# DeltaPavonis/cpp_raytracer

Hardware: AMD Instinct MI355X
Metric: Msamples/sec + achieved HBM GB/s, RTOW final scene at 1/2/4/8 MI355X (higher is better)
Workload: dtype f64; 1 GPU; rtow_final seed 42, 1200x800, 500 spp, max_depth 50 (BASELINE config 2); primitives=485, bvh_nodes=115, partition=whole frame on one GPU

## Files before the change

### cpp_raytracer_amd/__init__.py

```python
from __future__ import annotations

import ctypes as C
import struct
from dataclasses import dataclass
from pathlib import Path
from typing import Optional

import numpy as np

from . import _capi
from ._capi import (CRT_BOX, CRT_DIELECTRIC, CRT_DIFFUSE_LIGHT, CRT_LAMBERTIAN, CRT_METAL,
                    CRT_PARALLELOGRAM, CRT_SPHERE, HIT_DTYPE, MATERIAL_DTYPE, NODE_DTYPE,
                    OBJECT_DTYPE, CRT_BLOCK_STOPPED, FEATURE_DTYPE, BVHParams, Camera, CameraSettings, CrtError,
                    DenoiseParams, RenderStats, SceneInfo, Tiling, TraceParams, CRT_TRACE_ANY, CRT_TRACE_PLAIN,
                    RadianceParams, CRT_RADIANCE_PLAIN, ProbeParams, CRT_PROBE_SPHERE, CRT_PROBE_HEMISPHERE,
                    CRT_SH_RADIANCE, CRT_SH_IRRADIANCE, Lens, CRT_LENS_PINHOLE, CRT_LENS_ORTHOGRAPHIC,
                    CRT_LENS_EQUIRECT, CRT_LENS_FISHEYE, CRT_LENS_CUBE, check, lib)

__all__ = [
    "SceneData", "GpuScene", "CameraSettings", "Camera", "Tiling", "RenderStats", "CrtError",
    "resolve_camera", "sample_seed", "rand_double", "device_count", "lib", "ppm_values", "write_ppm",
    "sample_chunk_len", "noise_estimate", "block_count", "adaptive_update", "CRT_BLOCK_STOPPED",
    "DenoiseParams", "FEATURE_DTYPE", "denoise_params", "pixel_variance", "denoise",
    "TraceParams", "CRT_TRACE_ANY", "CRT_TRACE_PLAIN", "HIT_DTYPE",
# ... 174 lines not shown
    def save(self, path) -> None:
        Path(path).write_bytes(self.to_bytes())

    @classmethod
    def from_bytes(cls, b: bytes) -> "SceneData":
        if b[:4] != SCENE_MAGIC:
            raise CrtError("not a CRTS scene file")
        ver, nm, no = struct.unpack_from("<IQQ", b, 4)
        if ver != SCENE_VERSION:
            raise CrtError(f"CRTS version {ver} unsupported")
        off = 4 + struct.calcsize("<IQQ")
        cs = CameraSettings.from_buffer_copy(b[off:off + C.sizeof(CameraSettings)])
        off += C.sizeof(CameraSettings)
        mats = np.frombuffer(b, MATERIAL_DTYPE, nm, off).copy()
        off += nm * MATERIAL_DTYPE.itemsize
        objs = np.frombuffer(b, OBJECT_DTYPE, no, off).copy()
        return cls(mats, objs, cs)

    @classmethod
    def load(cls, path) -> "SceneData":
        return cls.from_bytes(Path(path).read_bytes())


def resolve_camera(settings: CameraSettings, base_seed: int = 0) -> Camera:
    cam = Camera()
    check(lib().crt_camera_resolve(C.byref(settings), C.byref(cam)), "crt_camera_resolve")
    cam.base_seed = base_seed & 0xFFFFFFFF
    return cam


def camera_with(settings: CameraSettings, **kw) -> CameraSettings:
    cs = CameraSettings.from_buffer_copy(_settings_bytes(settings))
    for k, v in kw.items():
        setattr(cs, k, v)
    return cs


class GpuScene:

    def __init__(self, data: SceneData, num_buckets: int = 32, max_prims_in_node: int = 12,
                 linear: bool = False, build_device: Optional[int] = None):
        self.data = data
        self._h = C.c_void_p()
        mats = np.ascontiguousarray(data.materials, dtype=MATERIAL_DTYPE)
        objs = np.ascontiguousarray(data.objects, dtype=OBJECT_DTYPE)
        prm = BVHParams(num_buckets, max_prims_in_node, int(linear),
                        0 if build_device is None else build_device + 1)
        check(lib().crt_scene_create(mats.ctypes.data, len(mats), objs.ctypes.data, len(objs),
                                     C.byref(prm), C.byref(self._h)), "crt_scene_create")

    def close(self) -> None:
        if self._h:
            lib().crt_scene_destroy(self._h)
            self._h = C.c_void_p()

    def __del__(self):
        try:
            self.close()
        except Exception:
            pass

    @property
    def handle(self) -> C.c_void_p:
        return self._h

    def info(self) -> SceneInfo:
        si = SceneInfo()
        check(lib().crt_scene_info_get(self._h, C.byref(si)), "crt_scene_info_get")
        return si

    def export_bvh(self) -> tuple[np.ndarray, np.ndarray]:
        si = self.info()
        nodes = np.zeros(si.num_nodes, NODE_DTYPE)
        order = np.zeros(si.num_primitives, np.uint32)
        check(lib().crt_scene_export_bvh(self._h, nodes.ctypes.data, order.ctypes.data),
              "crt_scene_export_bvh")
        return nodes, order

    def launch_plan(self, kernel="render") -> _capi.LaunchPlan:
        k = {"render": _capi.CRT_PLAN_RENDER, "trace": _capi.CRT_PLAN_TRACE, "radiance": _capi.CRT_PLAN_RADIANCE}.get(kernel, kernel)
        p = _capi.LaunchPlan()
        check(lib().crt_launch_plan(self._h, int(k), C.byref(p)), "crt_launch_plan")
        return p

    def upload(self, device: int = 0) -> None:
        check(lib().crt_scene_upload(self._h, device), f"crt_scene_upload(device={device})")

    def device_image(self, device: int = 0) -> np.ndarray:
        out = np.zeros(self.info().device_bytes, np.uint8)
        check(lib().crt_scene_image(self._h, device, out.ctypes.data, out.nbytes),
              f"crt_scene_image(device={device})")
        return out

    def render_async(self, device: int, cam: Camera, out_ptr: int, stream: int = 0,
                     tiling: Optional[Tiling] = None) -> None:
        t = C.byref(tiling) if tiling is not None else None
        check(lib().crt_render_async(self._h, device, C.byref(cam), t, C.c_void_p(out_ptr),
                                     C.c_void_p(stream)), "crt_render_async")

    def render_pass(self, device: int, cam: Camera, first: int, count: int, sum_ptr: int,
                    noise_ptr: int = 0, out_ptr: int = 0, stream: int = 0,
                    tiling: Optional[Tiling] = None) -> None:
        t = C.byref(tiling) if tiling is not None else None
        check(lib().crt_render_pass_async(self._h, device, C.byref(cam), t, first, count,
                                          C.c_void_p(sum_ptr), C.c_void_p(noise_ptr or None),
                                          C.c_void_p(out_ptr or None), C.c_void_p(stream)),
              "crt_render_pass_async")

    def render_pass_masked(self, device: int, cam: Camera, first: int, count: int, sum_ptr: int,
                           noise_ptr: int, out_ptr: int, blocks_ptr: int, active_hint: int = 0,
                           stream: int = 0, tiling: Optional[Tiling] = None) -> None:
        t = C.byref(tiling) if tiling is not None else None
        check(lib().crt_render_pass_masked_async(self._h, device, C.byref(cam), t, first, count,
                                                 C.c_void_p(sum_ptr), C.c_void_p(noise_ptr or None),
                                                 C.c_void_p(out_ptr or None), C.c_void_p(blocks_ptr or None),
                                                 min(active_hint, 0xFFFFFFFF), C.c_void_p(stream)),
              "crt_render_pass_masked_async")

    def render_adaptive(self, cam: Camera, threshold: float, min_samples: int = 0, samples_per_pass: int = 0,
                        callback=None, num_devices: int = 1,
                        preview: bool = False) -> tuple[np.ndarray, np.ndarray, int]:
        out = np.empty((cam.image_h, cam.image_w, 3), np.float64)
        counts = np.zeros(((cam.image_h + 3) // 4, (cam.image_w + 15) // 16), np.uint32)
        raised = []

        def trampoline(_user, done, total, active, blocks, h_rgb):
            try:
                return 1 if callback(done, total, active, blocks, out if h_rgb else None) else 0
            except BaseException as e:
                raised.append(e)
                return 1

        fn = _capi.ADAPTIVE_FN(trampoline) if callback is not None else _capi.ADAPTIVE_FN()
        prm = _capi.AdaptiveParams(threshold, min_samples, samples_per_pass,
                                   _capi.CRT_PROGRESS_PREVIEW if preview else 0, 0)
        rendered = C.c_uint64(0)
        rc = lib().crt_render_adaptive(self._h, C.byref(cam), num_devices, C.byref(prm), fn, None,
                                       out.ctypes.data, counts.ctypes.data, C.byref(rendered))
        if raised:
            raise raised[0]
        check(rc, "crt_render_adaptive")
        return out, counts, int(rendered.value)

    adaptive_update = staticmethod(adaptive_update)
    block_count = staticmethod(block_count)
    pixel_variance = staticmethod(pixel_variance)
    denoise = staticmethod(denoise)

    def render_features(self, device: int, cam: Camera, feat_ptr: int, stream: int = 0,
                        tiling: Optional[Tiling] = None) -> None:
        t = C.byref(tiling) if tiling is not None else None
        check(lib().crt_render_features_async(self._h, device, C.byref(cam), t, C.c_void_p(feat_ptr or None),
                                              C.c_void_p(stream)), "crt_render_features_async")

    def render_denoised(self, cam: Camera, params: Optional[DenoiseParams] = None, threshold: Optional[float] = None,
                        min_samples: int = 0, samples_per_pass: int = 0, device: int = 0,
                        noisy: bool = False, *, num_devices: int = 1, callback=None, preview: bool = False,
                        counts: bool = False):
        out = np.empty((cam.image_h, cam.image_w, 3), np.float64)
        raw = np.empty_like(out) if noisy else None
        prm = params if params is not None else denoise_params()
        rendered = C.c_uint64(0)
        if num_devices == 1 and callback is None and not preview and not counts:
            ad = _capi.AdaptiveParams(threshold, min_samples, samples_per_pass, 0, 0) if threshold is not None else None
            check(lib().crt_render_denoised(self._h, device, C.byref(cam), C.byref(ad) if ad is not None else None,
                                            C.byref(prm), raw.ctypes.data if noisy else None, out.ctypes.data,
# ... 357 lines not shown
```

### cpp_raytracer_amd/_capi.py

```python
from __future__ import annotations

import ctypes as C
import os
from pathlib import Path

import numpy as np

PKG_DIR = Path(__file__).resolve().parent
LIB_PATH = Path(os.environ.get("CRT_LIB", PKG_DIR / "lib" / "libcrt_hip.so"))

CRT_LAMBERTIAN, CRT_METAL, CRT_DIELECTRIC, CRT_DIFFUSE_LIGHT = 1, 2, 3, 4
CRT_SPHERE, CRT_PARALLELOGRAM, CRT_BOX = 1, 2, 3

D3 = C.c_double * 3


class Material(C.Structure):
    _fields_ = [("kind", C.c_uint32), ("reserved", C.c_uint32), ("color", D3), ("param", C.c_double)]


class Object(C.Structure):
    _fields_ = [("kind", C.c_uint32), ("material", C.c_uint32), ("v", C.c_double * 9)]


# ... 142 lines not shown
ADAPTIVE_FN = C.CFUNCTYPE(C.c_int, C.c_void_p, C.c_uint32, C.c_uint32, C.c_uint32, C.c_uint32, C.c_void_p)
DENOISED_FN = C.CFUNCTYPE(C.c_int, C.c_void_p, C.c_uint32, C.c_uint32, C.c_uint32, C.c_uint32, C.c_void_p, C.c_void_p)
CRT_BLOCK_W, CRT_BLOCK_H, CRT_BLOCK_STOPPED = 16, 4, 0x80000000
EXPORTS = {
    "crt_abi_version": (C.c_int, []),
    "crt_last_error": (C.c_char_p, []),
    "crt_build_info": (C.c_char_p, []),
    "crt_device_count": (C.c_int, [P(C.c_int)]),
    "crt_free": (None, [C.c_void_p]),
    "crt_sample_seed": (C.c_uint32, [C.c_uint32, C.c_uint32, C.c_uint32]),
    "crt_rand_double": (C.c_double, [P(C.c_uint32), C.c_double, C.c_double]),
    "crt_scene_build_named": (C.c_int, [C.c_char_p, C.c_uint32, C.c_int, P(P(Material)), P(C.c_size_t),
                                        P(P(Object)), P(C.c_size_t), P(CameraSettings)]),
    "crt_scene_create": (C.c_int, [C.c_void_p, C.c_size_t, C.c_void_p, C.c_size_t, P(BVHParams),
                                   P(C.c_void_p)]),
    "crt_scene_info_get": (C.c_int, [C.c_void_p, P(SceneInfo)]),
    "crt_scene_export_bvh": (C.c_int, [C.c_void_p, C.c_void_p, C.c_void_p]),
    "crt_scene_upload": (C.c_int, [C.c_void_p, C.c_int]),
    "crt_scene_image": (C.c_int, [C.c_void_p, C.c_int, C.c_void_p, C.c_size_t]),
    "crt_scene_destroy": (None, [C.c_void_p]),
    "crt_camera_resolve": (C.c_int, [P(CameraSettings), P(Camera)]),
    "crt_render_async": (C.c_int, [C.c_void_p, C.c_int, P(Camera), P(Tiling), C.c_void_p, C.c_void_p]),
    "crt_sample_chunk_len": (C.c_uint32, [C.c_uint32]),
    "crt_render_pass_async": (C.c_int, [C.c_void_p, C.c_int, P(Camera), P(Tiling), C.c_uint32, C.c_uint32,
                                        C.c_void_p, C.c_void_p, C.c_void_p, C.c_void_p]),
    "crt_noise_estimate": (C.c_int, [C.c_int, C.c_void_p, C.c_size_t, C.c_uint32, C.c_uint32,
                                     P(C.c_double), P(C.c_double), C.c_void_p]),
    "crt_render_progressive": (C.c_int, [C.c_void_p, P(Camera), C.c_int, C.c_uint32, C.c_uint32, PROGRESS_FN,
                                         C.c_void_p, C.c_void_p, P(C.c_uint32)]),
    "crt_block_count": (C.c_size_t, [C.c_uint32, C.c_uint32]),
    "crt_render_pass_masked_async": (C.c_int, [C.c_void_p, C.c_int, P(Camera), P(Tiling), C.c_uint32, C.c_uint32,
                                               C.c_void_p, C.c_void_p, C.c_void_p, C.c_void_p, C.c_uint32,
                                               C.c_void_p]),
    "crt_adaptive_update": (C.c_int, [C.c_int, P(Camera), P(Tiling), C.c_void_p, C.c_void_p, C.c_uint32,
                                      C.c_double, C.c_uint32, P(C.c_uint32), C.c_void_p]),
    "crt_render_adaptive": (C.c_int, [C.c_void_p, P(Camera), C.c_int, P(AdaptiveParams), ADAPTIVE_FN, C.c_void_p,
                                      C.c_void_p, C.c_void_p, P(C.c_uint64)]),
    "crt_render_features_async": (C.c_int, [C.c_void_p, C.c_int, P(Camera), P(Tiling), C.c_void_p, C.c_void_p]),
    "crt_pixel_variance_async": (C.c_int, [C.c_int, P(Camera), P(Tiling), C.c_void_p, C.c_void_p, C.c_uint32,
                                           C.c_void_p, C.c_void_p]),
    "crt_denoise_async": (C.c_int, [C.c_int, C.c_uint32, C.c_uint32, C.c_void_p, C.c_void_p, C.c_void_p,
                                    P(DenoiseParams), C.c_void_p, C.c_void_p, C.c_void_p]),
    "crt_render_denoised": (C.c_int, [C.c_void_p, C.c_int, P(Camera), P(AdaptiveParams), P(DenoiseParams),
                                      C.c_void_p, C.c_void_p, P(C.c_uint64)]),
    "crt_render_denoised_devices": (C.c_int, [C.c_void_p, P(Camera), C.c_int, P(AdaptiveParams), P(DenoiseParams),
                                              DENOISED_FN, C.c_void_p, C.c_void_p, C.c_void_p, C.c_void_p,
                                              P(C.c_uint64)]),
    "crt_render_count": (C.c_int, [C.c_void_p, C.c_int, P(Camera), P(Tiling), P(RenderStats)]),
    "crt_render": (C.c_int, [C.c_void_p, P(Camera), C.c_int, C.c_void_p, P(RenderStats)]),
    "crt_render_ppm": (C.c_int, [C.c_void_p, P(Camera), C.c_int, C.c_void_p, P(RenderStats)]),
    "crt_closest_hits": (C.c_int, [C.c_void_p, C.c_int, C.c_void_p, C.c_size_t, C.c_double, C.c_double,
                                   C.c_void_p]),
    "crt_trace_async": (C.c_int, [C.c_void_p, C.c_int, C.c_void_p, C.c_size_t, C.c_void_p, P(TraceParams),
                                  C.c_void_p, C.c_void_p, C.c_void_p]),
    "crt_trace": (C.c_int, [C.c_void_p, C.c_int, C.c_void_p, C.c_size_t, C.c_void_p, P(TraceParams), C.c_void_p,
                            C.c_void_p]),
    "crt_radiance_async": (C.c_int, [C.c_void_p, C.c_int, C.c_void_p, C.c_size_t, C.c_void_p, P(RadianceParams),
                                     C.c_void_p, C.c_void_p]),
    "crt_radiance": (C.c_int, [C.c_void_p, C.c_int, C.c_void_p, C.c_size_t, C.c_void_p, P(RadianceParams),
                               C.c_void_p]),
    "crt_camera_rays_async": (C.c_int, [C.c_int, P(Camera), P(Tiling), C.c_uint32, C.c_uint32, C.c_void_p,
                                        C.c_void_p, C.c_void_p]),
    "crt_probe_rays_async": (C.c_int, [C.c_int, C.c_void_p, C.c_void_p, C.c_size_t, P(ProbeParams), C.c_void_p,
                                       C.c_void_p, C.c_void_p]),
    "crt_probes_async": (C.c_int, [C.c_void_p, C.c_int, C.c_void_p, C.c_void_p, C.c_size_t, P(ProbeParams),
                                   C.c_void_p, C.c_void_p]),
    "crt_probes": (C.c_int, [C.c_void_p, C.c_int, C.c_void_p, C.c_void_p, C.c_size_t, P(ProbeParams), C.c_void_p]),
    "crt_sh_eval_async": (C.c_int, [C.c_int, C.c_void_p, C.c_size_t, C.c_void_p, C.c_void_p, C.c_size_t, C.c_uint32,
                                    C.c_void_p, C.c_void_p]),
    "crt_lens_rays_async": (C.c_int, [C.c_int, P(Camera), P(Lens), C.c_uint32, C.c_uint32, C.c_void_p, C.c_void_p,
                                      C.c_void_p]),
    "crt_render_lens_async": (C.c_int, [C.c_void_p, C.c_int, P(Camera), P(Lens), C.c_void_p, C.c_void_p]),
    "crt_render_lens": (C.c_int, [C.c_void_p, C.c_int, P(Camera), P(Lens), C.c_void_p]),
    "crt_render_lens_pass_async": (C.c_int, [C.c_void_p, C.c_int, P(Camera), P(Lens), C.c_uint32, C.c_uint32,
                                             C.c_void_p, C.c_void_p, C.c_void_p, C.c_void_p, C.c_uint32, C.c_void_p]),
    "crt_lens_centre_rays_async": (C.c_int, [C.c_int, P(Camera), P(Lens), C.c_void_p, C.c_void_p]),
    "crt_lens_features_async": (C.c_int, [C.c_void_p, C.c_int, P(Camera), P(Lens), C.c_void_p, C.c_void_p]),
    "crt_render_lens_passes": (C.c_int, [C.c_void_p, C.c_int, P(Camera), P(Lens), P(AdaptiveParams), P(DenoiseParams),
                                         DENOISED_FN, C.c_void_p, C.c_void_p, C.c_void_p, C.c_void_p, P(C.c_uint64)]),
    "crt_ppm_values": (C.c_int, [C.c_int, C.c_void_p, C.c_size_t, C.c_void_p, C.c_void_p]),
    "crt_ppm_write": (C.c_int, [C.c_char_p, C.c_uint32, C.c_uint32, C.c_void_p]),
    "crt_render_guard": (C.c_int, [C.c_void_p, C.c_int, P(C.c_uint64), C.c_int]),
    "crt_launch_plan": (C.c_int, [C.c_void_p, C.c_uint32, P(LaunchPlan)]),
}


class CrtError(RuntimeError):
    pass


_lib = None


def lib() -> C.CDLL:
    global _lib
    if _lib is None:
        if not LIB_PATH.exists():
            raise CrtError(f"{LIB_PATH} is missing: run __graft_entry__.build() "
                           "(make -C cpp_raytracer_amd); there is no fallback path")
        h = C.CDLL(str(LIB_PATH), mode=os.RTLD_NOW | C.RTLD_GLOBAL)
        for name, (res, args) in EXPORTS.items():
            f = getattr(h, name)
            f.restype = res
            f.argtypes = args
        _lib = h
    return _lib


def check(rc: int, what: str = "") -> None:
    if rc != 0:
        msg = lib().crt_last_error().decode(errors="replace")
        raise CrtError(f"{what or 'crt'} failed ({rc}): {msg}")
```

### cpp_raytracer_amd/csrc/crt_device.hip

```cpp
#include <hip/hip_runtime.h>

#define CRT_HD __host__ __device__ __forceinline__

#include <algorithm>
#include <atomic>
#include <cmath>
#include <cstdio>
#include <cstring>
#include <limits>
#include <string>
#include <mutex>
#include <thread>
#include <type_traits>
#include <vector>

#include "crt_internal.h"
#include "crt_hip_util.h"
#include "crt_rows.h"
#include "crt_ray_class.h"
#include "crt_schlick.h"

#pragma clang fp contract(off)

namespace crt {

namespace dev {

#ifndef CRT_BLOCK
#define CRT_BLOCK 256
#endif
constexpr int kBlock = CRT_BLOCK;
#ifndef CRT_TILE_W
#define CRT_TILE_W 16
#endif
constexpr uint32_t kTileW = CRT_TILE_W, kTileH = 64 / CRT_TILE_W;
constexpr int kManyWaves = 5;
#ifndef CRT_PAIR_WALK
#define CRT_PAIR_WALK 1
#endif
constexpr double kScale = 1 / static_cast<double>(4294967295u - 1);

typedef double Dvec2 __attribute__((ext_vector_type(2)));
typedef uint32_t Uvec4 __attribute__((ext_vector_type(4)));

struct SceneView {
    const DevNode* nodes;
    const DevNodeF* fnodes;
    uint32_t ntop;
    const uint32_t* refs;
    const DevSphere* spheres;
    const DevSpherePair* spair;
    uint32_t spair_lds;
    const uint32_t* sphere_mat;
    const DevQuad* quads;
    const uint32_t* quad_mat;
    const DevMaterial* mats;
    const DevQuadF* quadf;
    const DevMaterial* sphere_mrec;
    const DevMaterial* quad_mrec;
    uint32_t quadf_lds;
    const DevQuadBox* quadbox;
    uint32_t refs_lds, spheres_lds, quads_lds;
    uint32_t inv64_lds;
    unsigned long long* guard;
};

struct CamView {
    double o[3], p00[3], pdx[3], pdy[3], ddx[3], ddy[3];
    double defocus_angle;
    double bg[3];
    double t_min;
    double inv_spp;
    uint32_t w, h, spp, max_depth, base_seed;
};

struct Work {
    uint32_t owned_rows;
    uint32_t row_block, tile_count, tile_index;
    uint32_t col0, k0, bw, bh;
    uint32_t tiles_x, tiles_y, tiles;
    uint32_t chunks, chunk_len;
    uint32_t s0;
    uint32_t* queue;
    uint32_t segments;
    uint32_t n_items, bulk_items;
    uint32_t item_chunks, groups, bulk_chunks, tail_chunks;
    uint32_t rb_shift;
    uint32_t lds_nodes, lds_refs, lds_spheres, lds_quads, lds_quadf, lds_stack;
    uint32_t bytes_nodes, bytes_refs, bytes_spheres, bytes_quads, bytes_quadf;
    uint32_t lds_sph64, bytes_sph64;
    uint32_t sphere_only;
    uint32_t exact_slab;
    uint32_t ntop;
    uint32_t sentinel;
    uint32_t lds_cam;
    uint32_t lds_acc;
    uint32_t lds_inv64;
    uint32_t packed;
    uint32_t count_spec, round_counters;
    uint32_t f32_ok;
    uint32_t pair_walk;
    uint32_t spheres_f32;
    uint32_t quads_f32;
    uint32_t quads_flat;
    float tmin32;
};

struct Counters {
    unsigned long long rays, nodes, sphere_tests, quad_tests;
    unsigned long long cyc_walk, cyc_leaf, cyc_shade, cyc_total;
    unsigned long long cyc_tail;
    unsigned long long it_walk, it_leaf, it_shade;
    unsigned long long slow_nodes, it_slow;
    unsigned long long cand, it_cand;
    unsigned long long rounds, round_walkers, round_leaves, round_done, shade_rounds;
    unsigned long long cyc_draw, cyc_init;
};

struct LaneCounters {
    uint32_t rays, nodes, sphere_tests, quad_tests;
    uint32_t it_walk, it_leaf, it_shade;
    uint32_t slow_nodes, it_slow;
    uint32_t cand, it_cand;
};

__device__ __forceinline__ void flush_counts(LaneCounters& c, Counters* t) {
    using ull = unsigned long long;
    atomicAdd(&t->rays, static_cast<ull>(c.rays));
    atomicAdd(&t->nodes, static_cast<ull>(c.nodes));
    atomicAdd(&t->sphere_tests, static_cast<ull>(c.sphere_tests));
    atomicAdd(&t->quad_tests, static_cast<ull>(c.quad_tests));
    atomicAdd(&t->it_walk, static_cast<ull>(c.it_walk));
    atomicAdd(&t->it_leaf, static_cast<ull>(c.it_leaf));
    atomicAdd(&t->it_shade, static_cast<ull>(c.it_shade));
    atomicAdd(&t->slow_nodes, static_cast<ull>(c.slow_nodes));
    atomicAdd(&t->it_slow, static_cast<ull>(c.it_slow));
    atomicAdd(&t->cand, static_cast<ull>(c.cand));
    atomicAdd(&t->it_cand, static_cast<ull>(c.it_cand));
    c = LaneCounters{};
}

__device__ __forceinline__ bool wave_leader() {
    const uint64_t m = __ballot(1);
    return (threadIdx.x & 63) == static_cast<uint32_t>(__ffsll(static_cast<long long>(m)) - 1);
}

#ifndef CRT_WATCHDOG
#define CRT_WATCHDOG 0
#endif
#if CRT_WATCHDOG
__device__ unsigned long long crt_wd_deadline;
#define CRT_WD(id, a, b)                                                                                   \
    do {                                                                                                   \
        if (wall_clock64() > *(volatile unsigned long long*)&crt_wd_deadline) {                            \
            if (wave_leader())                                                                             \
                printf("crt watchdog: block %u wave %u loop %d a %u b %u\n", blockIdx.x, threadIdx.x >> 6,  \
                       (int)(id), (unsigned)(a), (unsigned)(b));                                            \
            __builtin_amdgcn_endpgm();                                                                     \
        }                                                                                                  \
    } while (0)
#else
#define CRT_WD(id, a, b) do {} while (0)
#endif

__device__ __forceinline__ double rnd(uint32_t& s, double lo, double hi) {
    s = 1664525u * s + 1013904223u;
    return lo + (hi - lo) * static_cast<double>(s) * kScale;
}
__device__ __forceinline__ double rnd_pm1(uint32_t& s) {
    s = 1664525u * s + 1013904223u;
    return static_cast<double>(s) * (2 * kScale) + -1.0;
}
__device__ __forceinline__ double rnd_01(uint32_t& s) {
    s = 1664525u * s + 1013904223u;
    return static_cast<double>(s) * kScale;
}

__device__ __forceinline__ uint32_t sample_seed(uint32_t base, uint32_t pixel, uint32_t sample) {
    uint64_t z = (static_cast<uint64_t>(pixel) << 32) | sample;
    z += static_cast<uint64_t>(base) * 0x9E3779B97F4A7C15ull;
// ... 538 lines not shown
__device__ __forceinline__ bool slab64_inv(GlobalNode* p, const double o[3], uint32_t inv_lds, double tmin,
                                           double tmax) {
    NodeLines nd;
    node_lines(p, nd);
    typedef __attribute__((address_space(3))) const double LdsDoubleC;
    uint32_t t = threadIdx.x;
    asm volatile("" : "+v"(t));
    LdsDoubleC* q = (LdsDoubleC*)static_cast<uintptr_t>(inv_lds + t * 8);
    const double inv[3] = {q[0], q[kBlock], q[2 * kBlock]};
    const Dvec2 bx = nd.b[0], by = nd.b[1], bz = nd.b[2];
    const double x0 = (bx.x - o[0]) * inv[0], x1 = (bx.y - o[0]) * inv[0];
    const double y0 = (by.x - o[1]) * inv[1], y1 = (by.y - o[1]) * inv[1];
    const double z0 = (bz.x - o[2]) * inv[2], z1 = (bz.y - o[2]) * inv[2];
    const double near = fmax(fmax(fmin(x0, x1), fmin(y0, y1)), fmin(z0, z1));
    const double far = fmin(fmin(fmax(x0, x1), fmax(y0, y1)), fmax(z0, z1));
    return (near <= far) & (near < tmax) & (far > tmin);
}

struct NodeF {
    Uvec4 q0;
    Uvec4 q1;
};
typedef __attribute__((address_space(3))) const NodeF LdsNodeF;
typedef __attribute__((address_space(1))) const NodeF GlobalNodeF;
template <bool TOP, bool LS>
__device__ __forceinline__ void fetch_nodef(const SceneView& S, uint32_t cur, Uvec4& q0, Uvec4& q1) {
    if (LS) {
        LdsNodeF* p = (LdsNodeF*)static_cast<uintptr_t>(cur);
        q0 = p->q0;
        q1 = p->q1;
    } else if (TOP) {
        const uint64_t hbm = __ballot(cur >= S.ntop);
        uint64_t save;
        asm volatile(
            "s_and_saveexec_b64 %[save], %[hbm]\n\t"
            "s_cbranch_execz 1f\n\t"
            "global_load_dwordx4 %[q0], %[cur], %[base]\n\t"
            "global_load_dwordx4 %[q1], %[cur], %[base] offset:16\n"
            "1:\n\t"
            "s_andn2_b64 exec, %[save], %[hbm]\n\t"
            "s_cbranch_execz 2f\n\t"
            "ds_read_b128 %[q0], %[cur]\n\t"
            "ds_read_b128 %[q1], %[cur] offset:16\n"
            "2:\n\t"
            "s_mov_b64 exec, %[save]\n\t"
            "s_waitcnt vmcnt(0) lgkmcnt(0)"
            : [q0] "=&v"(q0), [q1] "=&v"(q1), [save] "=&s"(save)
            : [cur] "v"(cur), [hbm] "s"(hbm), [base] "s"(S.fnodes)
            : "memory");
    } else {
        GlobalNodeF* p = (GlobalNodeF*)(reinterpret_cast<const char*>(S.fnodes) + cur);
        q0 = p->q0;
        q1 = p->q1;
    }
}

typedef uint32_t Uvec2 __attribute__((ext_vector_type(2)));
template <bool TOP, bool LS>
__device__ __forceinline__ Uvec2 fetch_nodef_words(const SceneView& S, uint32_t cur) {
    typedef __attribute__((address_space(3))) const Uvec2 LdsU2;
    typedef __attribute__((address_space(1))) const Uvec2 GlobalU2;
    if (LS) return *(LdsU2*)static_cast<uintptr_t>(cur + 24);
    if (!TOP) return *(GlobalU2*)(reinterpret_cast<const char*>(S.fnodes) + cur + 24);
    const uint64_t hbm = __ballot(cur >= S.ntop);
    uint64_t save;
    Uvec2 w;
    asm volatile(
        "s_and_saveexec_b64 %[save], %[hbm]\n\t"
        "s_cbranch_execz 1f\n\t"
        "global_load_dwordx2 %[w], %[cur], %[base] offset:24\n"
        "1:\n\t"
        "s_andn2_b64 exec, %[save], %[hbm]\n\t"
        "s_cbranch_execz 2f\n\t"
        "ds_read_b64 %[w], %[cur] offset:24\n"
        "2:\n\t"
        "s_mov_b64 exec, %[save]\n\t"
        "s_waitcnt vmcnt(0) lgkmcnt(0)"
        : [w] "=&v"(w), [save] "=&s"(save)
        : [cur] "v"(cur), [hbm] "s"(hbm), [base] "s"(S.fnodes)
        : "memory");
    return w;
}

template <typename SE, bool COUNT, bool EXACT, bool TOP, bool LS, bool GS, bool SPEC, bool INVL = false, bool G2 = true>
__device__ __forceinline__ void walk(const SceneView& S, Stack<SE>& st, const double o[3], const double d[3],
                                     double tmin, float tmin32, Trav& R, LaneCounters& ctr) {
    const ptrdiff_t stride = static_cast<ptrdiff_t>(st.stride);
    SE* const empty = st.base - stride;
    SE* tp = st.base + (static_cast<ptrdiff_t>(R.sp) - 1) * stride;
    uint32_t cur = R.cur;
    uint32_t w0, w1;
    bool stop;
    if (EXACT) {
        double dx = d[0], dy = d[1], dz = d[2];
        asm volatile("" : "+v"(dx), "+v"(dy), "+v"(dz));
        const double inv[3] = {1 / dx, 1 / dy, 1 / dz};
        do {
            NodeLines nd;
            node_lines(node64(S, cur), nd);
            const Uvec4 meta = nd.meta;
            const uint32_t top = *tp;
            if (COUNT) {
                if (meta.y != kSentinelCount) ctr.nodes++;
                if (wave_leader()) ctr.it_walk++;
            }
            const bool nx = R.neg & 1u, ny = (R.neg >> 1) & 1u, nz = (R.neg >> 2) & 1u;
            const double bx0 = nx ? nd.b[0].y : nd.b[0].x, bx1 = nx ? nd.b[0].x : nd.b[0].y;
            const double by0 = ny ? nd.b[1].y : nd.b[1].x, by1 = ny ? nd.b[1].x : nd.b[1].y;
            const double bz0 = nz ? nd.b[2].y : nd.b[2].x, bz1 = nz ? nd.b[2].x : nd.b[2].y;
            double xtmin = (bx0 - o[0]) * inv[0];
            double xtmax = (bx1 - o[0]) * inv[0];
            const double ytmin = (by0 - o[1]) * inv[1];
            const double ytmax = (by1 - o[1]) * inv[1];
            const double ztmin = (bz0 - o[2]) * inv[2];
            const double ztmax = (bz1 - o[2]) * inv[2];
            const bool c1 = !(xtmin > ytmax || ytmin > xtmax);
            if (ytmin > xtmin) xtmin = ytmin;
            if (ytmax < xtmax) xtmax = ytmax;
            const bool c2 = !(xtmin > ztmax || ztmin > xtmax);
            if (ztmin > xtmin) xtmin = ztmin;
            if (ztmax < xtmax) xtmax = ztmax;
            const bool enter = (c1 & c2 & (xtmin < R.tmax) & (xtmax > tmin)) |
                               (meta.y != 0 && (meta.w & kNodeAlways) != 0) | (meta.y == kSentinelCount);
            const bool inner = enter & (meta.y == 0);
            const bool far_first = (R.neg >> meta.z) & 1u;
            const uint32_t left = meta.w << kNodeFShift, right = meta.x << kNodeFShift;
            tp[stride] = static_cast<SE>(far_first ? left : right);
            stop = enter ^ inner;
            cur = inner ? (far_first ? right : left) : top;
            tp += inner ? stride : -stride;
            w0 = meta.x;
            w1 = meta.y == kSentinelCount ? kSentinelW1 : (kLeafFlagF | meta.y);
        } while (!stop);
    } else if (SPEC) {
        bool run = true, nopend = true;
        uint32_t pref = ~0u, pcur = 0;
        do {
            CRT_WD(4, cur, static_cast<uint32_t>(tp - empty));
            if (run) {
                Uvec4 q0, q1;
                fetch_nodef<TOP, LS>(S, cur, q0, q1);
                w0 = q1.z;
                w1 = q1.w;
                const uint32_t top = *tp;
                if (COUNT) {
                    if (w1 != kSentinelW1) ctr.nodes++;
                    if (wave_leader()) ctr.it_walk++;
                }
                const float x0 = __builtin_fmaf(__uint_as_float(q0.x), R.inv32[0], -R.oinv32[0]);
                const float x1 = __builtin_fmaf(__uint_as_float(q0.y), R.inv32[0], -R.oinv32[0]);
                const float y0 = __builtin_fmaf(__uint_as_float(q0.z), R.inv32[1], -R.oinv32[1]);
                const float y1 = __builtin_fmaf(__uint_as_float(q0.w), R.inv32[1], -R.oinv32[1]);
                const float z0 = __builtin_fmaf(__uint_as_float(q1.x), R.inv32[2], -R.oinv32[2]);
                const float z1 = __builtin_fmaf(__uint_as_float(q1.y), R.inv32[2], -R.oinv32[2]);
                const float lo = vmax3(vmin(x0, x1), vmin(y0, y1), vmax_s(vmin(z0, z1), tmin32));
                const float hi = vmin3(vmax(x0, x1), vmax(y0, y1), vmin(vmax(z0, z1), R.tmax32));
                const float gap = hi - lo;
                const float th = __builtin_fmaf(vmax_abs(lo, hi), 0x1p-19f, R.marg);
                bool enter = gap > 0.f;
                const bool unc = !(fabsf(gap) > th);
                if (__builtin_expect(__ballot(unc) != 0, 0)) {
                    if (COUNT && wave_leader()) ctr.it_slow++;
                    if (unc) {
                        if (COUNT) ctr.slow_nodes++;
                        enter = INVL ? slab64_inv(node64(S, cur), o, S.inv64_lds, tmin, R.tmax)
                                     : slab64(node64(S, cur), o, d, tmin, R.tmax);
                    }
                }
                const bool inner = enter & (w1 < kLeafFlagF);
                const uint32_t near = w1 | (__builtin_amdgcn_ubfe(R.neg, w0, 1) << kNodeFShift);
                tp[stride] = static_cast<SE>(near ^ (1u << kNodeFShift));
                const bool reached = enter & !inner;
                const bool park = reached & (!nopend | (!G2 && w1 == kSentinelW1));
                pref = (reached & nopend) ? cur : pref;
                pcur = park ? cur : pcur;
                run = !park;
                cur = inner ? near : top;
                tp += inner ? stride : -stride;
            }
            nopend = pref == ~0u;
        } while (__ballot(nopend) != 0);
        if (!run) {
            cur = pcur;
            tp += stride;
        }
        {
            const Uvec2 w = fetch_nodef_words<TOP, LS>(S, pref);
            w0 = w.x;
            w1 = w.y;
        }
        R.state = w1 == kSentinelW1 ? kDone : kLeaf;
        R.first = w0;
        R.count = w1 & ~kLeafFlagF;
        R.cur = cur;
        R.sp = static_cast<int32_t>(static_cast<uint32_t>(tp - empty)) / static_cast<int32_t>(st.stride);
        return;
    } else {
        do {
            CRT_WD(5, cur, static_cast<uint32_t>(tp - empty));
            Uvec4 q0, q1;
            fetch_nodef<TOP, LS>(S, cur, q0, q1);
            w0 = q1.z;
            w1 = q1.w;
            const uint32_t top = *tp;
            if (COUNT) {
                if (w1 != kSentinelW1) ctr.nodes++;
                if (wave_leader()) ctr.it_walk++;
            }
            const float x0 = __builtin_fmaf(__uint_as_float(q0.x), R.inv32[0], -R.oinv32[0]);
            const float x1 = __builtin_fmaf(__uint_as_float(q0.y), R.inv32[0], -R.oinv32[0]);
            const float y0 = __builtin_fmaf(__uint_as_float(q0.z), R.inv32[1], -R.oinv32[1]);
            const float y1 = __builtin_fmaf(__uint_as_float(q0.w), R.inv32[1], -R.oinv32[1]);
            const float z0 = __builtin_fmaf(__uint_as_float(q1.x), R.inv32[2], -R.oinv32[2]);
            const float z1 = __builtin_fmaf(__uint_as_float(q1.y), R.inv32[2], -R.oinv32[2]);
            const float lo = vmax3(vmin(x0, x1), vmin(y0, y1), vmax_s(vmin(z0, z1), tmin32));
            const float hi = vmin3(vmax(x0, x1), vmax(y0, y1), vmin(vmax(z0, z1), R.tmax32));
            const float gap = hi - lo;
            const float th = __builtin_fmaf(vmax_abs(lo, hi), 0x1p-19f, R.marg);
            bool enter = gap > 0.f;
            const bool unc = !(fabsf(gap) > th);
            if (__builtin_expect(__ballot(unc) != 0, 0)) {
                if (COUNT && wave_leader()) ctr.it_slow++;
                if (unc) {
                    if (COUNT) ctr.slow_nodes++;
                    enter = INVL ? slab64_inv(node64(S, cur), o, S.inv64_lds, tmin, R.tmax)
                                 : slab64(node64(S, cur), o, d, tmin, R.tmax);
                }
            }
            const bool inner = enter & (w1 < kLeafFlagF);
            const uint32_t near = w1 | (__builtin_amdgcn_ubfe(R.neg, w0, 1) << kNodeFShift);
            tp[stride] = static_cast<SE>(near ^ (1u << kNodeFShift));
            stop = enter ^ inner;
            cur = inner ? near : top;
            tp += inner ? stride : -stride;
        } while (!stop);
    }
    R.state = w1 == kSentinelW1 ? kDone : kLeaf;
    R.first = w0;
    R.count = w1 & ~kLeafFlagF;
    R.cur = cur;
    R.sp = static_cast<int32_t>(static_cast<uint32_t>(tp - empty)) / static_cast<int32_t>(st.stride);
}


constexpr uint32_t kTokAlone = 1u;

__device__ __forceinline__ uint32_t vsel(uint64_t m, uint32_t a, uint32_t b) {
    uint32_t r;
    asm("v_cndmask_b32_e64 %0, %1, %2, %3" : "=v"(r) : "v"(b), "v"(a), "s"(m));
    return r;
}

template <bool TOP>
__device__ __forceinline__ void fetch_two(const SceneView& S, uint32_t f, uint32_t g, Uvec4& a0, Uvec4& a1, Uvec4& b0,
                                          Uvec4& b1) {
    if (TOP) {
        const uint64_t hbm = __ballot(f >= S.ntop);
        uint64_t save;
        asm volatile(
            "s_and_saveexec_b64 %[save], %[hbm]\n\t"
            "s_cbranch_execz 1f\n\t"
            "global_load_dwordx4 %[a0], %[f], %[base]\n\t"
            "global_load_dwordx4 %[a1], %[f], %[base] offset:16\n\t"
            "global_load_dwordx4 %[b0], %[g], %[base]\n\t"
            "global_load_dwordx4 %[b1], %[g], %[base] offset:16\n"
            "1:\n\t"
            "s_andn2_b64 exec, %[save], %[hbm]\n\t"
            "s_cbranch_execz 2f\n\t"
            "ds_read_b128 %[a0], %[f]\n\t"
            "ds_read_b128 %[a1], %[f] offset:16\n\t"
            "ds_read_b128 %[b0], %[g]\n\t"
            "ds_read_b128 %[b1], %[g] offset:16\n"
            "2:\n\t"
            "s_mov_b64 exec, %[save]\n\t"
            "s_waitcnt vmcnt(0) lgkmcnt(0)"
            : [a0] "=&v"(a0), [a1] "=&v"(a1), [b0] "=&v"(b0), [b1] "=&v"(b1), [save] "=&s"(save)
            : [f] "v"(f), [g] "v"(g), [hbm] "s"(hbm), [base] "s"(S.fnodes)
            : "memory");
    } else {
        GlobalNodeF* qa = (GlobalNodeF*)(reinterpret_cast<const char*>(S.fnodes) + f);
        GlobalNodeF* qb = (GlobalNodeF*)(reinterpret_cast<const char*>(S.fnodes) + g);
        a0 = qa->q0;
        a1 = qa->q1;
        b0 = qb->q0;
        b1 = qb->q1;
    }
}

__device__ __forceinline__ void node_lohi(const Uvec4& q0, const Uvec4& q1, const Trav& R, float tmin32, float& lo,
                                          float& hi) {
    const float x0 = __builtin_fmaf(__uint_as_float(q0.x), R.inv32[0], -R.oinv32[0]);
    const float x1 = __builtin_fmaf(__uint_as_float(q0.y), R.inv32[0], -R.oinv32[0]);
    const float y0 = __builtin_fmaf(__uint_as_float(q0.z), R.inv32[1], -R.oinv32[1]);
    const float y1 = __builtin_fmaf(__uint_as_float(q0.w), R.inv32[1], -R.oinv32[1]);
    const float z0 = __builtin_fmaf(__uint_as_float(q1.x), R.inv32[2], -R.oinv32[2]);
    const float z1 = __builtin_fmaf(__uint_as_float(q1.y), R.inv32[2], -R.oinv32[2]);
    lo = vmax3(vmin(x0, x1), vmin(y0, y1), vmax_s(vmin(z0, z1), tmin32));
    hi = vmin3(vmax(x0, x1), vmax(y0, y1), vmin(vmax(z0, z1), R.tmax32));
}

template <typename SE, bool COUNT, bool TOP, bool INVL>
__device__ __forceinline__ void walk_pairs(const SceneView& S, Stack<SE>& st, const double o[3], const double d[3],
                                           double tmin, float tmin32, Trav& R, LaneCounters& ctr) {
    const ptrdiff_t stride = static_cast<ptrdiff_t>(st.stride);
    SE* const empty = st.base - stride;
    SE* tp = st.base + (static_cast<ptrdiff_t>(R.sp) - 1) * stride;
    uint32_t cur = R.cur;
    uint32_t run = 1;
    uint32_t pref = ~0u;
    uint64_t nop = __ballot(true);
    do {
        CRT_WD(7, cur, static_cast<uint32_t>(tp - empty));
        if (run) {
            const uint32_t f = cur & ~kTokAlone, g = f ^ 32u;
            Uvec4 a0, a1, b0, b1;
            fetch_two<TOP>(S, f, g, a0, a1, b0, b1);
            const uint32_t top = *tp;
            float lo1, hi1, lo2, hi2;
            node_lohi(a0, a1, R, tmin32, lo1, hi1);
            node_lohi(b0, b1, R, tmin32, lo2, hi2);
            const float g1 = hi1 - lo1, g2 = hi2 - lo2;
            const float t1 = __builtin_fmaf(vmax_abs(lo1, hi1), 0x1p-19f, R.marg);
            const float t2 = __builtin_fmaf(vmax_abs(lo2, hi2), 0x1p-19f, R.marg);
            const uint64_t two = __ballot(cur == f);
            uint64_t e1 = __ballot(g1 > 0.f), e2 = __ballot(g2 > 0.f) & two;
            const uint64_t u1 = __ballot(!(fabsf(g1) > t1)), u2 = two & __ballot(!(fabsf(g2) > t2));
            if (COUNT) {
                if (a1.w != kSentinelW1) ctr.nodes++;
                ctr.nodes += cur == f ? 1 : 0;
                if (wave_leader()) ctr.it_walk++;
            }
            if (__builtin_expect((u1 | u2) != 0, 0)) {
                if (COUNT && wave_leader()) ctr.it_slow++;
                const uint64_t me = 1ull << (threadIdx.x & 63);
                bool f1 = false, f2 = false;
                if (u1 & me) {
                    if (COUNT) ctr.slow_nodes++;
                    f1 = INVL ? slab64_inv(node64(S, f), o, S.inv64_lds, tmin, R.tmax) : slab64(node64(S, f), o, d, tmin, R.tmax);
                }
                if (u2 & me) {
                    if (COUNT) ctr.slow_nodes++;
                    f2 = INVL ? slab64_inv(node64(S, g), o, S.inv64_lds, tmin, R.tmax) : slab64(node64(S, g), o, d, tmin, R.tmax);
                }
                e1 = (e1 & ~u1) | __ballot(f1);
                e2 = (e2 & ~u2) | __ballot(f2);
            }
            const uint64_t i1 = __ballot(a1.w < kLeafFlagF), i2 = __ballot(b1.w < kLeafFlagF);
            const uint64_t both = e1 & e2, any = e1 | e2;
            const uint64_t xi = (e1 & i1) | (~e1 & i2);
            const uint64_t leaf = any & ~xi;
            const uint64_t park = leaf & ~nop;
            const uint64_t dp = (any & xi) | park;
            const uint32_t tok1 = vsel(i1, (__builtin_amdgcn_ubfe(R.neg, a1.z, 1) << kNodeFShift) | a1.w, cur | kTokAlone);
            const uint32_t tok2 = vsel(i2, (__builtin_amdgcn_ubfe(R.neg, b1.z, 1) << kNodeFShift) | b1.w, g | kTokAlone);
            const uint32_t tx = vsel(e1, tok1, tok2);
            pref = vsel(leaf & nop, tx, pref);
            tp[stride] = static_cast<SE>(tok2);
            cur = vsel(dp, tx, vsel(both, tok2, top));
            tp += static_cast<int32_t>(vsel(dp & both, 1u, vsel(~dp & ~both, ~0u, 0u))) * stride;
            run = vsel(park, 0u, 1u);
        }
        nop = __ballot(pref == ~0u);
    } while (nop != 0);
    {
        const Uvec2 w = fetch_nodef_words<TOP, false>(S, pref & ~kTokAlone);
        R.state = w.y == kSentinelW1 ? kDone : kLeaf;
        R.first = w.x;
        R.count = w.y & ~kLeafFlagF;
    }
    R.cur = cur;
    R.sp = static_cast<int32_t>(static_cast<uint32_t>(tp - empty)) / static_cast<int32_t>(st.stride);
}

template <typename SE, bool COUNT, bool TOP, bool LS, bool FAST = false, bool QONLY = false>
__device__ __forceinline__ void leaf_step(const SceneView& S, Stack<SE>& st, const double o[3],
                                              const double d[3], double tmin, float tmin32, bool sphere_only, bool pairs,
                                              bool qfilter, bool qflat, Trav& R, LaneCounters& ctr) {
    const uint2 range = make_uint2(R.first, R.count);
    const uint32_t end = range.x + range.y;
    const double ia = recip_a<FAST>(R.a), lo = lim_tmin(tmin, R.a);
    double hi = lim_tmax(R.tmax, R.a);
    if (!QONLY && pairs && range.y <= 32 && leaf_ray32_ok(o, d, R.a)) {
        LeafRay32 L;
        leaf_ray32(o, d, R.a, tmin, R.tmax, L);
        uint32_t cand = 0;
        const uint32_t nbits = (range.y + 1) & ~1u;
        if constexpr (LS) {
            for (uint32_t i = 0; i < range.y; i += 2) {
                if (COUNT) {
                    ctr.sphere_tests += i + 1 < range.y ? 2 : 1;
                    if (wave_leader()) ctr.it_leaf += 2;
                }
                cand = sphere_pair_candidates(cand, pair_at((LdsPair*)static_cast<uintptr_t>(S.spair_lds + ((range.x + i) << 5))), L);
            }
        } else {
            for (uint32_t i = 0; i < range.y; i += 2) {
                if (COUNT) {
                    ctr.sphere_tests += i + 1 < range.y ? 2 : 1;
                    if (wave_leader()) ctr.it_leaf += 2;
                }
                cand = sphere_pair_candidates(cand, pair_at((GlobalPair*)(S.spair + range.x + i)), L);
            }
        }
        cand &= ~(range.y & 1u);
        while (cand) {
            CRT_WD(6, cand, range.y);
            if (COUNT) {
                ctr.cand++;
                if (wave_leader()) ctr.it_cand++;
            }
            const uint32_t b = 31 - __builtin_clz(cand);
            cand ^= 1u << b;
            const uint32_t i = range.x + (nbits - 1 - b);
            double t;
            if (hit_sphere<false>(sphere_at<LS>(S, i), o, d, R.a, ia, tmin, R.tmax, lo, hi, t)) {
                R.tmax = t;
                R.tmax32 = tmax_f32(t);
                hi = lim_tmax(t, R.a);
                R.ref = i;
                R.found = true;
            }
        }
    } else if (LS && qfilter && qflat && range.y <= 32) {
        uint32_t cand = 0;
        const uint32_t base = S.quadf_lds + (range.x << 5);
        const uint32_t g = lds_u32(base + 28);
        const uint32_t e0 = g & 0xffu, e1 = e0 + ((g >> 8) & 0xffu);
        uint32_t i = 0;
        const auto filter = [&](auto axis) {
            if (COUNT) {
                ctr.quad_tests++;
                if (wave_leader()) ctr.it_leaf++;
            }
            LdsNodeF* p = (LdsNodeF*)static_cast<uintptr_t>(base + (i << 5));
            const Uvec4 q0 = p->q0, q1 = p->q1;
            const float b[6] = {__uint_as_float(q0.x), __uint_as_float(q0.y), __uint_as_float(q0.z),
                                __uint_as_float(q0.w), __uint_as_float(q1.x), __uint_as_float(q1.y)};
            cand |= static_cast<uint32_t>(flat_axis_candidate<decltype(axis)::value, DevMinMax>(b, R.inv32, R.oinv32, tmin32, R.tmax32, R.marg)) << q1.z;
        };
        for (; i < e0; ++i) filter(std::integral_constant<int, 0>{});
        for (; i < e1; ++i) filter(std::integral_constant<int, 1>{});
        for (; i < range.y; ++i) filter(std::integral_constant<int, 2>{});
        while (cand) {
            CRT_WD(6, cand, range.y);
            if (COUNT) {
                ctr.cand++;
                if (wave_leader()) ctr.it_cand++;
            }
            const uint32_t i = range.x + static_cast<uint32_t>(__builtin_ctz(cand));
            cand &= cand - 1;
            double t;
            if (hit_quad(lds_rec<DevQuad>(S.quads_lds + (i << 7)), o, d, tmin, R.tmax, t)) {
                R.tmax = t;
                R.tmax32 = tmax_f32(t);
                R.ref = kRefQuad | i;
                R.found = true;
            }
        }
    } else if (LS && qfilter && !qflat && range.y <= 32 && quad_ray32_ok(o, d)) {
        QuadRay32 L;
        quad_ray32(o, d, tmin, R.tmax, L);
        uint32_t cand = 0;
        for (uint32_t i = 0; i < range.y; ++i) {
            if (COUNT) {
                ctr.quad_tests++;
                if (wave_leader()) ctr.it_leaf++;
            }
            const DevQuadF q = LS ? lds_rec<DevQuadF>(S.quadf_lds + ((range.x + i) << 6)) : quadf_global(S.quadf + range.x + i);
            cand |= static_cast<uint32_t>(quad_candidate(q, L, [](float x) { return __builtin_amdgcn_rcpf(x); })) << i;
        }
        while (cand) {
            CRT_WD(6, cand, range.y);
            if (COUNT) {
                ctr.cand++;
                if (wave_leader()) ctr.it_cand++;
            }
            const uint32_t i = range.x + static_cast<uint32_t>(__builtin_ctz(cand));
            cand &= cand - 1;
            double t;
            bool h;
            if constexpr (LS) h = hit_quad(lds_rec<DevQuad>(S.quads_lds + (i << 7)), o, d, tmin, R.tmax, t);
            else h = hit_quad(S.quads[i], o, d, tmin, R.tmax, t);
            if (h) {
                R.tmax = t;
                R.tmax32 = tmax_f32(t);
                R.ref = kRefQuad | i;
                R.found = true;
            }
        }
    } else if (!QONLY && sphere_only) {
        DevSphere cur = sphere_at<LS>(S, range.x);
        for (uint32_t i = range.x; i < end; ++i) {
            const DevSphere nxt = sphere_at<LS>(S, i + 1);
            if (COUNT) {
                ctr.sphere_tests++;
                if (wave_leader()) ctr.it_leaf++;
            }
            double t;
            if (hit_sphere(cur, o, d, R.a, ia, tmin, R.tmax, lo, hi, t)) {
                R.tmax = t;
                R.tmax32 = tmax_f32(t);
                hi = lim_tmax(t, R.a);
                R.ref = i;
                R.found = true;
            }
            cur = nxt;
        }
    } else {
        for (uint32_t i = range.x; i < end; ++i) {
            const uint32_t ref = LS ? lds_u32(S.refs_lds + (i << 2)) : S.refs[i];
            double t;
            bool h;
            if (COUNT && wave_leader()) ctr.it_leaf++;
            if (QONLY || (ref & kRefQuad)) {
                if (COUNT) ctr.quad_tests++;
                if constexpr (LS) h = hit_quad(lds_rec<DevQuad>(S.quads_lds + ((ref & ~kRefQuad) << 7)), o, d, tmin, R.tmax, t);
                else h = hit_quad(S.quads[ref & ~kRefQuad], o, d, tmin, R.tmax, t);
            } else {
                if (COUNT) ctr.sphere_tests++;
                if constexpr (LS) h = hit_sphere(lds_rec<DevSphere>(S.spheres_lds + (ref << 5)), o, d, R.a, ia, tmin, R.tmax, lo, hi, t);
                else h = hit_sphere(S.spheres[ref], o, d, R.a, ia, tmin, R.tmax, lo, hi, t);
            }
            if (h) {
                R.tmax = t;
                R.tmax32 = tmax_f32(t);
                hi = lim_tmax(t, R.a);
                R.ref = ref;
                R.found = true;
            }
        }
    }
    R.state = R.sp < 0 ? kDone : kWalk;
}

__device__ __forceinline__ uint32_t owned_row(const Work& w, uint32_t k) {
    if (w.rb_shift < 32) {
        const uint32_t blk = k >> w.rb_shift, in = k & ((1u << w.rb_shift) - 1);
        return ((blk * w.tile_count + w.tile_index) << w.rb_shift) | in;
    }
    const uint32_t blk = k / w.row_block, in = k % w.row_block;
    return (blk * w.tile_count + w.tile_index) * w.row_block + in;
}

struct Path {
    double o[3], d[3];
    double T[3];
    uint32_t depth;
    uint32_t rng;
};

__device__ __forceinline__ void start_path(const CamView& C, uint32_t row, uint32_t col, uint32_t rng, Path& P) {
    if (C.defocus_angle <= 0) {
        P.o[0] = C.o[0]; P.o[1] = C.o[1]; P.o[2] = C.o[2];
    } else {
        double vx, vy;
        do {
            vx = rnd_pm1(rng);
            vy = rnd_pm1(rng);
        } while (!(vx * vx + vy * vy + 0.0 * 0.0 < 1));
        P.o[0] = (C.o[0] + C.ddx[0] * vx) + C.ddy[0] * vy;
        P.o[1] = (C.o[1] + C.ddx[1] * vx) + C.ddy[1] * vy;
        P.o[2] = (C.o[2] + C.ddx[2] * vx) + C.ddy[2] * vy;
    }
    uint32_t ir = row, ic = col;
    asm volatile("" : "+v"(ir), "+v"(ic));
    const double fr = static_cast<double>(ir), fc = static_cast<double>(ic);
    const double uy = rnd(rng, -0.5, 0.5);
    const double ux = rnd(rng, -0.5, 0.5);
#pragma unroll
    for (int k = 0; k < 3; ++k) {
        const double center = (C.p00[k] + C.pdy[k] * fr) + C.pdx[k] * fc;
        const double sample = (center + C.pdx[k] * ux) + C.pdy[k] * uy;
        P.d[k] = sample - P.o[k];
        P.T[k] = 1;
    }
    P.depth = C.max_depth;
    P.rng = rng;
}

template <bool LS, bool SPH = false, bool QONLY = false, bool FAST = false>
__device__ __forceinline__ bool shade(const SceneView& S, const CamView& C, Path& P, bool hit,
                                      uint32_t ref, double t, double acc[3]) {
    if (!hit) {
        acc[0] = acc[0] + P.T[0] * C.bg[0];
        acc[1] = acc[1] + P.T[1] * C.bg[1];
        acc[2] = acc[2] + P.T[2] * C.bg[2];
        return true;
    }
    const DevMaterial& M = (QONLY || (!SPH && (ref & kRefQuad))) ? S.quad_mrec[ref & ~kRefQuad] : S.sphere_mrec[ref];
    double p[3], n[3];
    bool front;
    (void)hit_record<LS, true, SPH, QONLY>(S, ref, P.o, P.d, t, p, n, front, M.emit[0]);
    const uint32_t kind = M.kind;
    const bool lam = kind == CRT_LAMBERTIAN, met = kind == CRT_METAL, die = kind == CRT_DIELECTRIC;
    if (!(lam || met || die)) {
        acc[0] = acc[0] + P.T[0] * M.emit[0];
        acc[1] = acc[1] + P.T[1] * M.emit[1];
        acc[2] = acc[2] + P.T[2] * M.emit[2];
        return true;
    }
    double ux0 = 0, uy0 = 0, uz0 = 0;
    if (met || die) {
        const double il = recip_exact<FAST>(sqrt_exact<FAST>(P.d[0] * P.d[0] + P.d[1] * P.d[1] + P.d[2] * P.d[2]));
        ux0 = P.d[0] * il;
        uy0 = P.d[1] * il;
        uz0 = P.d[2] * il;
    }
    bool reflect = met;
    double cosv = 0, ratio = 0;
    if (die) {
        ratio = front ? M.color[0] : M.param;
        cosv = fmin((-ux0) * n[0] + (-uy0) * n[1] + (-uz0) * n[2], 1.);
        const double sinv = sqrt_exact<FAST>(1 - cosv * cosv);
        if (ratio * sinv > 1) {
            reflect = true;
        } else {
            const double r0 = front ? M.color[1] : M.color[2];
            const double pw = pow5(1 - cosv);
            const double u = rnd_01(P.rng);
            reflect = u < r0 + (1 - r0) * pw;
            if (__builtin_expect(schlick_undecided(u, r0, pw), 0)) atomicAdd(S.guard, 1ull);
        }
    }
    double rx = 0, ry = 0, rz = 0;
    if (lam || met) random_unit_vector<FAST>(P.rng, rx, ry, rz);
    double nd[3];
    if (reflect) {
        const double k2 = 2 * (ux0 * n[0] + uy0 * n[1] + uz0 * n[2]);
        nd[0] = ux0 - n[0] * k2;
        nd[1] = uy0 - n[1] * k2;
        nd[2] = uz0 - n[2] * k2;
        if (met) {
            nd[0] = nd[0] + rx * M.param;
            nd[1] = nd[1] + ry * M.param;
            nd[2] = nd[2] + rz * M.param;
            if (n[0] * nd[0] + n[1] * nd[1] + n[2] * nd[2] < 0) return true;
        }
    } else if (die) {
        const double px = (ux0 + n[0] * cosv) * ratio;
        const double py = (uy0 + n[1] * cosv) * ratio;
        const double pz = (uz0 + n[2] * cosv) * ratio;
        const double sq = -sqrt_exact<FAST>(fabs(1 - (px * px + py * py + pz * pz)));
        nd[0] = px + n[0] * sq;
        nd[1] = py + n[1] * sq;
        nd[2] = pz + n[2] * sq;
    } else {
        nd[0] = n[0] + rx; nd[1] = n[1] + ry; nd[2] = n[2] + rz;
        if (fabs(nd[0]) < 1e-8 && fabs(nd[1]) < 1e-8 && fabs(nd[2]) < 1e-8) {
            nd[0] = n[0]; nd[1] = n[1]; nd[2] = n[2];
        }
    }
    if (kind != CRT_DIELECTRIC) {
        P.T[0] = P.T[0] * M.color[0];
        P.T[1] = P.T[1] * M.color[1];
        P.T[2] = P.T[2] * M.color[2];
    }
    P.o[0] = p[0]; P.o[1] = p[1]; P.o[2] = p[2];
    P.d[0] = nd[0]; P.d[1] = nd[1]; P.d[2] = nd[2];
    P.depth -= 1;
    return false;
}

__device__ __forceinline__ void stage_lds(unsigned char* dst, const void* src, uint32_t bytes) {
    const uint4* s = static_cast<const uint4*>(src);
    uint4* d = reinterpret_cast<uint4*>(dst);
    for (uint32_t i = threadIdx.x; i < bytes / 16; i += kBlock) d[i] = s[i];
}

#ifndef CRT_WAVES_PER_EU
#define CRT_WAVES_PER_EU 4
#endif
#ifndef CRT_WAVES_PER_EU_LDS
#define CRT_WAVES_PER_EU_LDS 4
#endif
#ifndef CRT_SHADE_BATCH
#define CRT_SHADE_BATCH 48
#endif
constexpr int kShadeBatch = CRT_SHADE_BATCH;

constexpr bool kTopTreelet = true;
constexpr int kPrioWalk = 3, kPrioLeaf = 2, kPrioShade = 0, kPrioInit = 1;
template <int P>
__device__ __forceinline__ void set_prio() {
    if constexpr ((kPrioWalk | kPrioLeaf | kPrioShade | kPrioInit) != 0) __builtin_amdgcn_s_setprio(P);
}

template <typename SE, bool GSTACK, bool LSCENE, bool COUNT, int PM, bool W5, bool MASK = false>
__global__ __launch_bounds__(kBlock) __attribute__((amdgpu_waves_per_eu(W5 ? kManyWaves : LSCENE ? CRT_WAVES_PER_EU_LDS : CRT_WAVES_PER_EU, 8))) void render_kernel(
    SceneView Sg, CamView C, Work W, double* __restrict__ partial, SE* __restrict__ gstack,
    Counters* __restrict__ counters, const uint32_t* __restrict__ active) {
    extern __shared__ __attribute__((aligned(16))) unsigned char smem[];
    constexpr bool kSphOnly = PM == 0, kFlatOnly = PM == 2;
    constexpr bool kFast = kSphOnly && W5;
    SceneView S = Sg;
    if (LSCENE) {
        if (static_cast<uint32_t>(reinterpret_cast<uintptr_t>((LdsByte*)smem)) != 0) __builtin_trap();
        stage_lds(smem, Sg.fnodes, W.bytes_nodes);
        stage_lds(smem + W.lds_quads, Sg.quads, W.bytes_quads);
        S.quads = reinterpret_cast<const DevQuad*>(smem + W.lds_quads);
        S.quads_lds = W.lds_quads;
        if (W.quads_f32) {
            stage_lds(smem + W.lds_quadf, W.quads_flat ? static_cast<const void*>(Sg.quadbox) : Sg.quadf, W.bytes_quadf);
            S.quadf_lds = W.lds_quadf;
        }
        S.refs_lds = W.lds_refs;
        S.spheres_lds = W.spheres_f32 ? (W.bytes_sph64 ? W.lds_sph64 : ~0u) : W.lds_spheres;
        if (W.spheres_f32) {
            stage_lds(smem + W.lds_spheres, Sg.spair, W.bytes_spheres);
            if (W.bytes_sph64) stage_lds(smem + W.lds_sph64, Sg.spheres, W.bytes_sph64);
            S.spair_lds = W.lds_spheres;
        } else {
            stage_lds(smem + W.lds_refs, Sg.refs, W.bytes_refs);
            stage_lds(smem + W.lds_spheres, Sg.spheres, W.bytes_spheres);
            S.refs = reinterpret_cast<const uint32_t*>(smem + W.lds_refs);
            S.spheres = reinterpret_cast<const DevSphere*>(smem + W.lds_spheres);
        }
        __syncthreads();
    } else if (W.ntop) {
        if (static_cast<uint32_t>(reinterpret_cast<uintptr_t>((LdsByte*)smem)) != 0) __builtin_trap();
        stage_lds(smem, Sg.fnodes, W.ntop);
        S.ntop = W.ntop;
        __syncthreads();
    }
    if (threadIdx.x == 0) *reinterpret_cast<CamView*>(smem + W.lds_cam) = C;
#if CRT_WATCHDOG
    if (threadIdx.x == 0) atomicCAS(&crt_wd_deadline, 0ull, wall_clock64() + 300000000ull);
#endif
    __syncthreads();
    const CamView& CL = *reinterpret_cast<const CamView*>(smem + W.lds_cam);
    const float tmin32 = W.tmin32;
    const uint32_t lane = threadIdx.x & 63;
    LaneCounters ctr{};
    const unsigned long long t_start = COUNT ? wall_clock64() : 0;
    Stack<SE> st;
    if (GSTACK) {
        st.stride = gridDim.x * kBlock;
        st.base = gstack + (static_cast<size_t>(blockIdx.x) * kBlock + threadIdx.x) + 3 * static_cast<size_t>(st.stride);
    } else {
        st.base = reinterpret_cast<SE*>(smem + W.lds_stack) + threadIdx.x;
        st.stride = kBlock;
    }
    st.base[-static_cast<ptrdiff_t>(st.stride)] = static_cast<SE>(W.sentinel);
    st.base[-2 * static_cast<ptrdiff_t>(st.stride)] = static_cast<SE>(W.sentinel);
    uint32_t item_pos = 0, item_units = 0;
    const uint32_t q_tiles = MASK ? active[0] : W.tiles;
    uint32_t seg = blockIdx.x % W.segments, seg_tried = 0;
    uint32_t item_txy = 0, item_chunk = 0;
    uint32_t u_txy = 0, u_cp = 0, s = 0;
    double acc[3] = {0, 0, 0};
    constexpr bool kAccLds = kFast;
    typedef __attribute__((address_space(3))) double LdsDouble;
    LdsDouble* const acc_l = (LdsDouble*)static_cast<uintptr_t>(W.lds_acc + threadIdx.x * 8);
    constexpr bool kInvLds = (kFlatOnly && LSCENE && W5) || (!LSCENE && !GSTACK);
    constexpr bool kPair = CRT_PAIR_WALK && !LSCENE;
    const bool pw = kPair && W.pair_walk && (!COUNT || W.count_spec);
    S.inv64_lds = W.lds_inv64;
    if (kAccLds) {
        acc_l[0] = 0;
        acc_l[kBlock] = 0;
        acc_l[2 * kBlock] = 0;
    }
    Path P;
    Trav R;
    R.state = kIdle;
    bool need = true, start = false, cont = false;
    uint32_t cw = 0, cl = 0, cs = 0;
    uint32_t cd = 0, ci = 0;
    unsigned long long t_first_idle = 0;
    while (true) {
        CRT_WD(1, item_pos, item_units);
        if (COUNT) cd -= static_cast<uint32_t>(wall_clock64());
        set_prio<kPrioInit>();
        while (true) {
            CRT_WD(2, item_pos, item_units);
            const uint64_t m = __ballot(need);
            if (m == 0) break;
            if (item_pos >= item_units) {
                const uint32_t leader = static_cast<uint32_t>(__ffsll(static_cast<long long>(m)) - 1);
                item_units = 0;
                item_pos = 0;
                while (seg < W.segments) {
                    const uint32_t t0 = static_cast<uint32_t>(static_cast<uint64_t>(q_tiles) * seg / W.segments);
                    const uint32_t t1 = static_cast<uint32_t>(static_cast<uint64_t>(q_tiles) * (seg + 1) / W.segments);
                    const uint32_t nt = t1 - t0, bulk = nt * W.groups;
                    uint32_t v = 0;
                    if (lane == leader) v = atomicAdd(W.queue + seg, 1u);
                    const uint32_t j = __builtin_amdgcn_readlane(v, leader);
                    if (j < nt * (W.groups + W.tail_chunks)) {
                        uint32_t tile;
                        if (j < bulk) {
                            tile = j / W.groups;
                            item_chunk = (j - tile * W.groups) * W.item_chunks;
                            item_units = 64 * W.item_chunks;
                        } else {
                            const uint32_t jt = j - bulk;
                            tile = jt / W.tail_chunks;
                            item_chunk = W.bulk_chunks + (jt - tile * W.tail_chunks);
                            item_units = 64;
                        }
                        tile += t0;
                        if (MASK) tile = active[1 + tile];
                        item_txy = (tile % W.tiles_x) | ((tile / W.tiles_x) << 16);
                        break;
                    }
                    if (++seg_tried >= W.segments) seg = W.segments;
                    else seg = seg + 1 == W.segments ? 0 : seg + 1;
                }
            }
            if (item_units == 0) {
                need = false;
                break;
            }
            const uint32_t take = min(static_cast<uint32_t>(__popcll(m)), item_units - item_pos);
            const uint32_t r = __builtin_amdgcn_mbcnt_hi(static_cast<uint32_t>(m >> 32),
                                                         __builtin_amdgcn_mbcnt_lo(static_cast<uint32_t>(m), 0u));
            if (need && r < take) {
                const uint32_t uu = item_pos + r, pix = uu & 63, chunk = item_chunk + (uu >> 6);
                u_txy = item_txy;
                u_cp = (chunk << 6) | pix;
                const uint32_t col = (item_txy & 0xffffu) * kTileW + pix % kTileW, k = (item_txy >> 16) * kTileH + pix / kTileW;
                if (chunk < W.chunks && col < W.bw && k < W.bh) {
                    s = W.s0 + chunk * W.chunk_len;
                    if (C.max_depth > 0) {
                        need = false;
                        start = true;
                    } else if (!COUNT) {
                        double* dst = partial + (static_cast<size_t>(chunk) * W.bh * W.bw +
                                                 static_cast<size_t>(k) * W.bw + col) * 3;
                        dst[0] = 0;
                        dst[1] = 0;
                        dst[2] = 0;
                    }
                }
            }
            item_pos += take;
        }
        if (COUNT) {
            const uint32_t now = static_cast<uint32_t>(wall_clock64());
            cd += now;
            ci -= now;
        }
        if (start) {
            const uint32_t pix = u_cp & 63;
            const uint32_t col = W.col0 + (u_txy & 0xffffu) * kTileW + pix % kTileW;
            const uint32_t row = owned_row(W, W.k0 + (u_txy >> 16) * kTileH + pix / kTileW);
            start_path(CL, row, col, sample_seed(C.base_seed, row * C.w + col, s), P);
        }
        if (start || cont) {
            trav_init(P.o, P.d, W.f32_ok != 0, R);
            const bool tok = kPair && pw && !(R.neg & kZeroDir);
            st.base[-static_cast<ptrdiff_t>(st.stride)] = static_cast<SE>(W.sentinel | (tok ? kTokAlone : 0u));
            if (!kFlatOnly) st.base[-2 * static_cast<ptrdiff_t>(st.stride)] = static_cast<SE>(W.sentinel | (tok ? kTokAlone : 0u));
            if (tok) R.cur = kTokAlone;
            if (kInvLds) {
                uint32_t t = threadIdx.x;
                asm volatile("" : "+v"(t));
                LdsDouble* const inv_l = (LdsDouble*)static_cast<uintptr_t>(W.lds_inv64 + t * 8);
                inv_l[0] = 1 / P.d[0];
                inv_l[kBlock] = 1 / P.d[1];
                inv_l[2 * kBlock] = 1 / P.d[2];
            }
            if (COUNT) ctr.rays++;
        }
        start = false;
        cont = false;
        if (COUNT) ci += static_cast<uint32_t>(wall_clock64());
        while (true) {
            CRT_WD(3, R.state, R.cur);
            if (COUNT && W.round_counters) {
                const unsigned long long nw = __popcll(__ballot(R.state == kWalk));
                if (wave_leader()) {
                    atomicAdd(&counters->rounds, 1ull);
                    atomicAdd(&counters->round_walkers, nw);
                }
            }
            if (COUNT) cw -= static_cast<uint32_t>(wall_clock64());
            set_prio<kPrioWalk>();
            if (kPair && pw) {
                if (__ballot(R.state == kWalk && (R.neg & kZeroDir)) != 0) {
                    if (R.state == kWalk && (R.neg & kZeroDir))
                        walk<SE, COUNT, true, kTopTreelet && !LSCENE, LSCENE, GSTACK, false>(S, st, P.o, P.d, C.t_min, tmin32, R, ctr);
                }
                if (R.state == kWalk && !(R.neg & kZeroDir))
                    walk_pairs<SE, COUNT, kTopTreelet && !LSCENE, kInvLds>(S, st, P.o, P.d, C.t_min, tmin32, R, ctr);
            } else if (!W.exact_slab && __ballot(R.state == kWalk && (R.neg & kZeroDir)) == 0) {
                if (R.state == kWalk) {
                    if (!COUNT || W.count_spec)
                        walk<SE, COUNT, false, kTopTreelet && !LSCENE, LSCENE, GSTACK, true, kInvLds, !kFlatOnly>(S, st, P.o, P.d, C.t_min, tmin32, R, ctr);
                    else
                        walk<SE, COUNT, false, kTopTreelet && !LSCENE, LSCENE, GSTACK, false, kInvLds>(S, st, P.o, P.d, C.t_min, tmin32, R, ctr);
                }
            } else {
                if (R.state == kWalk) walk<SE, COUNT, true, kTopTreelet && !LSCENE, LSCENE, GSTACK, false>(S, st, P.o, P.d, C.t_min, tmin32, R, ctr);
            }
            if (COUNT) cw += static_cast<uint32_t>(wall_clock64());
            set_prio<kPrioLeaf>();
            if (COUNT && W.round_counters) {
                const unsigned long long nl = __popcll(__ballot(R.state == kLeaf));
                if (wave_leader()) atomicAdd(&counters->round_leaves, nl);
            }
            if (COUNT) cl -= static_cast<uint32_t>(wall_clock64());
            if (R.state == kLeaf) leaf_step<SE, COUNT, kTopTreelet && !LSCENE, LSCENE, kFast, kFlatOnly>(S, st, P.o, P.d, C.t_min, tmin32, kSphOnly || (!kFlatOnly && W.sphere_only != 0), !kFlatOnly && W.spheres_f32 != 0, kFlatOnly || (!kSphOnly && W.quads_f32 != 0), kFlatOnly || (!kSphOnly && W.quads_flat != 0), R, ctr);
            if (COUNT) cl += static_cast<uint32_t>(wall_clock64());
            const uint64_t pending = __ballot(R.state == kWalk);
            const uint64_t finished = __ballot(R.state == kDone);
            const int nfin = __popcll(finished);
            if (COUNT && W.round_counters && wave_leader()) atomicAdd(&counters->round_done, static_cast<unsigned long long>(nfin));
            if (pending == 0 || nfin >= kShadeBatch) break;
        }
        const uint64_t m_done = __ballot(R.state == kDone);
        if (COUNT && t_first_idle == 0 && __ballot(R.state == kIdle) != 0) t_first_idle = wall_clock64();
        if (m_done == 0) break;
        if (COUNT) cs -= static_cast<uint32_t>(wall_clock64());
        set_prio<kPrioShade>();
        if (COUNT && W.round_counters && wave_leader()) atomicAdd(&counters->shade_rounds, 1ull);
        if (COUNT && ((ctr.rays | ctr.nodes | ctr.sphere_tests | ctr.quad_tests | ctr.it_walk | ctr.it_leaf |
                       ctr.it_shade | ctr.slow_nodes | ctr.it_slow | ctr.cand | ctr.it_cand) & 0x80000000u))
            flush_counts(ctr, counters);
        if (R.state == kDone) {
            if (COUNT && wave_leader()) ctr.it_shade++;
            double contrib[3] = {0, 0, 0};
            bool ended = shade<LSCENE, kSphOnly, kFlatOnly, kFast>(S, CL, P, R.found, R.ref, R.tmax, kAccLds ? contrib : acc);
            if (kAccLds && ended) {
                acc_l[0] = acc_l[0] + contrib[0];
                acc_l[kBlock] = acc_l[kBlock] + contrib[1];
                acc_l[2 * kBlock] = acc_l[2 * kBlock] + contrib[2];
            }
            if (!ended && P.depth == 0) ended = true;
            if (!ended) {
                cont = true;
            } else {
                const uint32_t chunk = u_cp >> 6;
                if (++s < min(C.spp, W.s0 + (chunk + 1) * W.chunk_len)) {
                    start = true;
                } else {
                    if (!COUNT) {
                        const uint32_t pix = u_cp & 63;
                        const uint32_t col = (u_txy & 0xffffu) * kTileW + pix % kTileW, k = (u_txy >> 16) * kTileH + pix / kTileW;
                        double* dst = partial + (static_cast<size_t>(chunk) * W.bh * W.bw +
                                                 static_cast<size_t>(k) * W.bw + col) * 3;
                        dst[0] = kAccLds ? acc_l[0] : acc[0];
                        dst[1] = kAccLds ? acc_l[kBlock] : acc[1];
                        dst[2] = kAccLds ? acc_l[2 * kBlock] : acc[2];
                    }
                    if (kAccLds) {
                        acc_l[0] = 0;
                        acc_l[kBlock] = 0;
                        acc_l[2 * kBlock] = 0;
                    }
                    acc[0] = 0;
                    acc[1] = 0;
                    acc[2] = 0;
                    need = true;
                }
                R.state = kIdle;
            }
        }
        if (COUNT) cs += static_cast<uint32_t>(wall_clock64());
    }
    if (COUNT) {
        using ull = unsigned long long;
        flush_counts(ctr, counters);
        if (lane == 0) {
            atomicAdd(&counters->cyc_walk, static_cast<ull>(cw));
            atomicAdd(&counters->cyc_leaf, static_cast<ull>(cl));
            atomicAdd(&counters->cyc_shade, static_cast<ull>(cs));
            atomicAdd(&counters->cyc_draw, static_cast<ull>(cd));
            atomicAdd(&counters->cyc_init, static_cast<ull>(ci));
            const unsigned long long t_end = wall_clock64();
            atomicAdd(&counters->cyc_total, t_end - t_start);
            atomicAdd(&counters->cyc_tail, t_first_idle ? t_end - t_first_idle : 0ull);
        }
    }
}

__global__ __launch_bounds__(256) void resolve_kernel(const double* __restrict__ partial,
                                                      double* __restrict__ out, Work W, uint32_t w,
                                                      uint32_t h, double inv_spp) {
    const uint64_t i = static_cast<uint64_t>(blockIdx.x) * 256 + threadIdx.x;
    const uint64_t band = static_cast<uint64_t>(W.bh) * W.bw;
    if (i >= band) return;
    const uint32_t k = W.k0 + static_cast<uint32_t>(i / W.bw), col = W.col0 + static_cast<uint32_t>(i % W.bw);
    const size_t pix = static_cast<size_t>(W.packed ? k : owned_row(W, k)) * w + col;
    const size_t plane = band * 3;
    double r = partial[i * 3 + 0], g = partial[i * 3 + 1], b = partial[i * 3 + 2];
// ... 792 lines not shown
                    walk<SE, false, false, kTopTreelet && !LSCENE, LSCENE, GSTACK, true, kInvLds>(S, st, P.o, P.d, tmin, tmin32, R, ctr);
            } else {
                if (R.state == kWalk) walk<SE, false, true, kTopTreelet && !LSCENE, LSCENE, GSTACK, false>(S, st, P.o, P.d, tmin, tmin32, R, ctr);
            }
            set_prio<kPrioLeaf>();
            if (R.state == kLeaf)
                leaf_step<SE, false, kTopTreelet && !LSCENE, LSCENE>(S, st, P.o, P.d, tmin, tmin32, kSphOnly || W.sphere_only != 0,
                                                                     W.spheres_f32 != 0, !kSphOnly && W.quads_f32 != 0,
                                                                     !kSphOnly && W.quads_flat != 0, R, ctr);
            const uint64_t pending = __ballot(R.state == kWalk);
            const int nfin = __popcll(__ballot(R.state == kDone));
            if (pending == 0 || nfin >= kShadeBatch) break;
        }
        if (__ballot(R.state == kDone) == 0) break;
        set_prio<kPrioShade>();
        if (R.state == kDone) {
            double acc[3] = {0, 0, 0};
            bool ended = shade<LSCENE, kSphOnly>(S, CL, P, R.found, R.ref, R.tmax, acc);
            if (!ended && P.depth == 0) ended = true;
            if (!ended) {
                cont = true;
            } else {
                double* dst = Q.rgb + 3 * static_cast<size_t>(ray);
                dst[0] = acc[0];
                dst[1] = acc[1];
                dst[2] = acc[2];
                R.state = kIdle;
                need = true;
            }
        }
    }
}

__global__ __launch_bounds__(256) void camera_rays_kernel(CamView C, Work W, uint32_t n, uint32_t s0, uint32_t ns,
                                                          double* __restrict__ rays, uint32_t* __restrict__ states) {
    const uint32_t i = blockIdx.x * 256 + threadIdx.x;
    if (i >= n) return;
    const uint32_t j = i / ns, s = s0 + i % ns;
    const uint32_t col = j % C.w, row = owned_row(W, j / C.w);
    Path P;
    start_path(C, row, col, sample_seed(C.base_seed, row * C.w + col, s), P);
    double* dst = rays + 6 * static_cast<size_t>(i);
    dst[0] = P.o[0]; dst[1] = P.o[1]; dst[2] = P.o[2];
    dst[3] = P.d[0]; dst[4] = P.d[1]; dst[5] = P.d[2];
    states[i] = P.rng;
}

__global__ __launch_bounds__(256) void pixel_variance_kernel(const double* __restrict__ noise,
                                                             const uint32_t* __restrict__ blocks, Work W, uint32_t w,
                                                             uint32_t n_pixels, uint32_t samples_done, uint32_t L_,
                                                             double* __restrict__ var_out) {
    const uint32_t i = blockIdx.x * 256 + threadIdx.x;
    if (i >= n_pixels) return;
    const uint32_t k = i / w, col = i % w;
    const size_t pix = static_cast<size_t>(W.packed ? k : owned_row(W, k)) * w + col;
    uint32_t n = samples_done;
    if (blocks) {
        const uint32_t tiles_x = (w + kTileW - 1) / kTileW;
        n = blocks[(k / kTileH) * tiles_x + col / kTileW] & ~CRT_BLOCK_STOPPED;
    }
    const uint32_t Ki = n / L_;
    const double K = static_cast<double>(Ki), L = static_cast<double>(L_);
    double v = 0;
    if (Ki >= 1) {
        const double t = noise[pix * 2 + 0], q = noise[pix * 2 + 1];
        const double m = t / (K * L);
        if (Ki == 1) {
            v = m * m;
        } else {
            const double var = q / (L * L) - K * m * m;
            v = (var > 0 ? var : 0.0) / (K * (K - 1));
        }
    }
    var_out[pix] = v;
}

}


static dev::SceneView view_of(const DeviceCopy& c) {
    dev::SceneView v{c.nodes, c.fnodes, 0, c.refs, c.spheres, c.spair, 0, c.sphere_mat, c.quads, c.quad_mat,
                     c.mats, c.quadf, c.sphere_mrec, c.quad_mrec, 0, c.quadbox};
    v.guard = c.guard;
    return v;
}

int device_count(int* n) {
    hipError_t e = hipGetDeviceCount(n);
    if (e != hipSuccess) {
        *n = 0;
        return fail(CRT_E_NODEVICE, std::string("hipGetDeviceCount: ") + hipGetErrorString(e));
    }
    return CRT_OK;
}

static int check_device(int device) {
    int n = 0;
    hipError_t e = hipGetDeviceCount(&n);
    if (e != hipSuccess || n == 0)
        return fail(CRT_E_NODEVICE, "no HIP device visible (the render path has no CPU fallback)");
    if (device < 0 || device >= n || device >= kMaxDevices)
        return fail(CRT_E_NODEVICE, "device " + std::to_string(device) + " out of range");
    return CRT_OK;
}

static size_t align256(size_t x) { return (x + 255) & ~size_t(255); }

static void stage_image(crt_scene* s) {
    const size_t n_nodes = s->num_dnodes, n_refs = s->num_prims;
    const size_t n_sp = s->num_spheres, n_q = s->num_quads, n_m = s->num_dmats;
    size_t off[kArrCount + 1];
    const size_t total = device_layout(s, off);
    BigVec<char>& img = s->image;
    img.resize(total);
    auto at = [&](int arr) { return img.data() + off[arr]; };
    for (int a = 0; a < kArrCount; ++a) {
        static const size_t kElem[kArrCount] = {sizeof(DevNode), sizeof(DevNodeF), 4, sizeof(DevSphere), sizeof(DevSpherePair),
                                                4, sizeof(DevQuad), sizeof(DevQuadF), sizeof(DevQuadBox), 4,
                                                sizeof(DevMaterial), sizeof(DevMaterial), sizeof(DevMaterial), 1};
        const size_t cnt[kArrCount] = {n_nodes, n_nodes, n_refs, n_sp, n_sp, n_sp, n_q, n_q, n_q, n_q, n_m, n_sp, n_q, 64};
        const size_t used = a == kArrGuard ? 0 : cnt[a] * kElem[a];
        std::memset(img.data() + off[a] + used, 0, off[a + 1] - off[a] - used);
    }
    auto put = [&](int arr, const void* src, size_t bytes) {
        char* dst = at(arr);
        const char* sp = static_cast<const char*>(src);
        parallel_for(bytes, size_t{1} << 22, [&](size_t a, size_t b) { std::memcpy(dst + a, sp + a, b - a); });
    };
    put(kArrNodes, s->dnodes.data(), n_nodes * sizeof(DevNode));
    put(kArrRefs, s->refs.data(), n_refs * 4);
    put(kArrSpheres, s->spheres.data(), n_sp * sizeof(DevSphere));
    put(kArrSphereMat, s->sphere_mat.data(), n_sp * 4);
    put(kArrQuads, s->quads.data(), n_q * sizeof(DevQuad));
    put(kArrQuadMat, s->quad_mat.data(), n_q * 4);
    put(kArrMats, s->dmats.data(), n_m * sizeof(DevMaterial));
    DevNodeF* fnodes = reinterpret_cast<DevNodeF*>(at(kArrFNodes));
    std::atomic<bool> f32_bad{false};
    parallel_for(n_nodes, 4096, [&](size_t a, size_t b) {
        bool bad = false;
        for (size_t i = a; i < b; ++i) bad = node_record(s->dnodes[i], static_cast<uint32_t>(i), fnodes[i]) || bad;
        if (bad) f32_bad = true;
    });
    DevSpherePair* spair = reinterpret_cast<DevSpherePair*>(at(kArrSpherePairs));
    std::atomic<bool> sph_bad{false};
    parallel_for(n_sp, 4096, [&](size_t a, size_t b) {
        bool bad = false;
        for (size_t i = a; i < b; ++i) {
            DevSpherePair& r = spair[i];
            bad = sphere_pair_half(s->spheres[i], r.cx[0], r.cy[0], r.cz[0], r.r2e[0]) || bad;
            if (i + 1 < n_sp) (void)sphere_pair_half(s->spheres[i + 1], r.cx[1], r.cy[1], r.cz[1], r.r2e[1]);
            else r.cx[1] = r.cy[1] = r.cz[1] = r.r2e[1] = 0;
        }
        if (bad) sph_bad = true;
    });
    DevQuadF* quadf = reinterpret_cast<DevQuadF*>(at(kArrQuadF));
    DevQuadBox* quadbox = reinterpret_cast<DevQuadBox*>(at(kArrQuadBox));
    std::atomic<bool> quads_bad{false}, flat_bad{false};
    parallel_for(n_q, 4096, [&](size_t a, size_t b) {
        bool qb = false, fb = false;
        for (size_t i = a; i < b; ++i) {
            const DevQuad& q = s->quads[i];
            if (!quad_record(q.v, q.s1, q.s2, q.sn, quadf[i])) qb = true;
            quadbox[i] = DevQuadBox{};
            if (!quad_flat_box(q.v, q.s1, q.s2, quadbox[i])) fb = true;
        }
        if (qb) quads_bad = true;
        if (fb) flat_bad = true;
    });
    std::atomic<bool> regroup_bad{false};
    if (!flat_bad && n_sp == 0 && n_q > 0) {
        parallel_for(n_nodes, 1 << 12, [&](size_t a, size_t b) {
            bool bad = false;
            for (size_t k = a; k < b; ++k) bad = regroup_leaf(s->dnodes[k], k, quadbox) || bad;
            if (bad) regroup_bad = true;
        });
    }
    DevMaterial* smrec = reinterpret_cast<DevMaterial*>(at(kArrSphereMrec));
    DevMaterial* qmrec = reinterpret_cast<DevMaterial*>(at(kArrQuadMrec));
    parallel_for(n_sp, 4096, [&](size_t a, size_t b) {
        for (size_t i = a; i < b; ++i) {
            smrec[i] = s->dmats[s->sphere_mat[i]];
            shading_consts(smrec[i], &s->spheres[i]);
        }
    });
    parallel_for(n_q, 4096, [&](size_t a, size_t b) {
        for (size_t i = a; i < b; ++i) {
            qmrec[i] = s->dmats[s->quad_mat[i]];
            shading_consts(qmrec[i], nullptr);
        }
    });
    s->image_f32_ok = !f32_bad;
    s->image_spheres_f32_ok = !sph_bad;
    s->image_quads_f32_ok = !quads_bad;
    s->image_quads_flat_ok = !flat_bad && !regroup_bad;
    s->staged = true;
}

struct CopyFlags {
    bool f32_ok, spheres_f32_ok, quads_f32_ok, quads_flat_ok;
};
static CopyFlags copy_flags(const crt_scene* s) {
    CopyFlags f;
    f.f32_ok = s->image_f32_ok && std::getenv("CRT_F64_NODES") == nullptr;
    f.spheres_f32_ok = s->image_spheres_f32_ok && std::getenv("CRT_F64_SPHERES") == nullptr;
    f.quads_f32_ok = s->image_quads_f32_ok && std::getenv("CRT_F64_QUADS") == nullptr;
    f.quads_flat_ok = s->image_quads_flat_ok && std::getenv("CRT_GENERIC_QUADS") == nullptr;
    return f;
}
static CopyFlags flags_of(const DeviceCopy& c) {
    return CopyFlags{c.f32_ok, c.spheres_f32_ok, c.quads_f32_ok, c.quads_flat_ok};
}

void device_bind_copy(crt_scene* s, int device, void* base, size_t total) {
    size_t off[kArrCount + 1];
    (void)device_layout(s, off);
    DeviceCopy& c = s->dev[device];
    const CopyFlags f = copy_flags(s);
    char* b = static_cast<char*>(base);
    c.base = base;
    c.bytes = total;
    c.nodes = reinterpret_cast<DevNode*>(b + off[kArrNodes]);
    c.fnodes = reinterpret_cast<DevNodeF*>(b + off[kArrFNodes]);
    c.f32_ok = f.f32_ok;
    c.refs = reinterpret_cast<uint32_t*>(b + off[kArrRefs]);
    c.spheres = reinterpret_cast<DevSphere*>(b + off[kArrSpheres]);
    c.spair = reinterpret_cast<DevSpherePair*>(b + off[kArrSpherePairs]);
    c.spheres_f32_ok = f.spheres_f32_ok;
    c.sphere_mat = reinterpret_cast<uint32_t*>(b + off[kArrSphereMat]);
    c.quads = reinterpret_cast<DevQuad*>(b + off[kArrQuads]);
    c.quadf = reinterpret_cast<DevQuadF*>(b + off[kArrQuadF]);
    c.quads_f32_ok = f.quads_f32_ok;
    c.quadbox = reinterpret_cast<DevQuadBox*>(b + off[kArrQuadBox]);
    c.quads_flat_ok = f.quads_flat_ok;
    c.quad_mat = reinterpret_cast<uint32_t*>(b + off[kArrQuadMat]);
    c.mats = reinterpret_cast<DevMaterial*>(b + off[kArrMats]);
    c.sphere_mrec = reinterpret_cast<DevMaterial*>(b + off[kArrSphereMrec]);
    c.quad_mrec = reinterpret_cast<DevMaterial*>(b + off[kArrQuadMrec]);
    c.guard = reinterpret_cast<unsigned long long*>(b + off[kArrGuard]);
    c.valid = true;
}

int device_upload(crt_scene* s, int device) {
    int rc = check_device(device);
    if (rc) return rc;
    std::lock_guard<std::mutex> lk(s->dev_mu[device]);
    DeviceCopy& c = s->dev[device];
    if (c.valid) return CRT_OK;
    if (s->num_dnodes >= (size_t{1} << (31 - kNodeFShift)))
        return fail(CRT_E_INVALID, "BVH too large for the device node layout");
    if (s->image_device < 0) {
        std::lock_guard<std::mutex> ls(s->mu);
        if (!s->staged) stage_image(s);
    }
    size_t off[kArrCount + 1];
    const size_t total = device_layout(s, off);
    DeviceGuard g(device);
    void* base = nullptr;
    HIP_TRY(hipMalloc(&base, total));
    hipError_t e = s->image_device >= 0
                       ? hipMemcpyPeer(base, device, s->dev[s->image_device].base, s->image_device, total)
                       : hipMemcpy(base, s->image.data(), total, hipMemcpyHostToDevice);
    if (e == hipSuccess && s->image_device >= 0)
        e = hipMemset(static_cast<char*>(base) + off[kArrGuard], 0, total - off[kArrGuard]);
    if (e != hipSuccess) {
        (void)hipFree(base);
        return fail(CRT_E_HIP, std::string("scene upload: ") + hipGetErrorString(e));
    }
    device_bind_copy(s, device, base, total);
    return CRT_OK;
}

int device_guard(crt_scene* s, int device, uint64_t* schlick_undecided, bool reset) {
    int rc = check_device(device);
    if (rc) return rc;
    std::lock_guard<std::mutex> lk(s->dev_mu[device]);
    DeviceCopy& c = s->dev[device];
    if (!c.valid) return fail(CRT_E_NOT_UPLOADED, "crt_render_guard: scene not uploaded to this device");
    DeviceGuard g(device);
    HIP_TRY(hipDeviceSynchronize());
    unsigned long long v = 0;
    HIP_TRY(hipMemcpy(&v, c.guard, sizeof v, hipMemcpyDeviceToHost));
    if (reset) HIP_TRY(hipMemset(c.guard, 0, sizeof v));
    *schlick_undecided = v;
    return CRT_OK;
}

int device_image(crt_scene* s, int device, void* host, size_t bytes) {
    int rc = device_upload(s, device);
    if (rc) return rc;
    const DeviceCopy& c = s->dev[device];
    if (bytes != c.bytes)
        return fail(CRT_E_INVALID, "crt_scene_image: bytes must be " + std::to_string(c.bytes));
    DeviceGuard g(device);
    HIP_TRY(hipMemcpy(host, c.base, c.bytes, hipMemcpyDeviceToHost));
    return CRT_OK;
}

void device_release(crt_scene* s) {
    for (int d = 0; d < kMaxDevices; ++d) {
        DeviceCopy& c = s->dev[d];
        if (!c.valid) continue;
        DeviceGuard g(d);
        (void)hipFree(c.base);
        if (c.ref_prim) (void)hipFree(c.ref_prim);
        c = DeviceCopy{};
    }
}

static dev::CamView cam_view(const crt_camera* cam) {
    dev::CamView v{};
    for (int k = 0; k < 3; ++k) {
        v.o[k] = cam->origin[k];
        v.p00[k] = cam->pixel00[k];
        v.pdx[k] = cam->pixel_delta_x[k];
        v.pdy[k] = cam->pixel_delta_y[k];
        v.ddx[k] = cam->defocus_disk_x[k];
        v.ddy[k] = cam->defocus_disk_y[k];
        v.bg[k] = cam->background[k];
    }
    v.defocus_angle = cam->defocus_angle;
    v.t_min = cam->t_min;
    v.inv_spp = 1 / static_cast<double>(cam->samples_per_pixel);
    v.w = cam->image_w;
    v.h = cam->image_h;
    v.spp = cam->samples_per_pixel;
    v.max_depth = cam->max_depth;
    v.base_seed = cam->base_seed;
    return v;
}

static size_t align16(size_t x) { return (x + 15) & ~size_t(15); }

constexpr size_t kAccBytes = 3 * dev::kBlock * sizeof(double);
constexpr size_t kInvBytes = 3 * dev::kBlock * sizeof(double);
constexpr size_t kLdsSceneBudget = 40 * 1024 * dev::kBlock / 256;
constexpr size_t kLdsStackBudget = 32 * 1024 * dev::kBlock / 256;
constexpr size_t kLdsBudget5 = 160 * 1024 * dev::kBlock / (64 * dev::kManyWaves * 4);
constexpr size_t kLdsPerBlock = 160 * 1024 * dev::kBlock / (256 * CRT_WAVES_PER_EU);

enum QueryClass { kQueryLdsScene, kQueryLdsStack, kQueryHbmStack };
struct Layout {
    QueryClass cls = kQueryLdsScene;
    bool w5 = false;
    size_t lds = 0;
    size_t stack_bytes = 0;
    size_t level = 0;
    size_t all_nodes = 0;
    size_t budget = 0;
};

static int render_prim_mode(const dev::Work& W, QueryClass cls) {
    return W.sphere_only ? 0 : (cls == kQueryLdsScene && W.quads_flat) ? 2 : 1;
}
static int query_prim_mode(const dev::Work& W) { return W.sphere_only ? 0 : 1; }

static size_t render_lds_tail(dev::Work& W, size_t lds, bool gstack, bool lscene, int pm, bool w5) {
    W.lds_cam = static_cast<uint32_t>(align16(lds));
    lds = W.lds_cam + align16(sizeof(dev::CamView));
    if (w5 && pm == 0) {
        W.lds_acc = static_cast<uint32_t>(align16(lds));
        lds = W.lds_acc + kAccBytes;
    }
    if ((lscene && pm == 2 && w5) || (!lscene && !gstack)) {
        W.lds_inv64 = static_cast<uint32_t>(align16(lds));
        lds = W.lds_inv64 + kInvBytes;
    }
    return lds;
}
static size_t trace_lds_tail(dev::Work& W, size_t lds, bool gstack, bool lscene) {
    if (gstack && lds % (2 * sizeof(DevNodeF))) lds += sizeof(DevNodeF);
    if (!lscene && !gstack) {
        W.lds_inv64 = static_cast<uint32_t>(align16(lds));
        lds = W.lds_inv64 + kInvBytes;
    }
    return lds;
}
static size_t radiance_lds_tail(dev::Work& W, size_t lds, bool gstack, bool lscene) {
    W.lds_cam = static_cast<uint32_t>(align16(lds));
    lds = W.lds_cam + align16(sizeof(dev::CamView));
    if (!lscene && !gstack) {
        W.lds_inv64 = static_cast<uint32_t>(align16(lds));
        lds = W.lds_inv64 + kInvBytes;
    }
    return lds;
}
static size_t gstack_levels(const crt_scene* s) { return static_cast<size_t>(s->depth) + 4; }

static void class_flags(const crt_scene* s, const CopyFlags& c, bool f32_ok, bool filters, dev::Work& W) {
    W.f32_ok = f32_ok ? 1u : 0u;
    W.sphere_only = (s->num_quads == 0 && s->num_spheres != 0) ? 1u : 0u;
    W.spheres_f32 = (W.sphere_only && c.spheres_f32_ok && filters) ? 1u : 0u;
    W.quads_f32 = (s->num_spheres == 0 && s->num_quads != 0 && c.quads_f32_ok && filters) ? 1u : 0u;
    W.quads_flat = (W.quads_f32 && c.quads_flat_ok && W.f32_ok) ? 1u : 0u;
    W.exact_slab = (s->exact_slab || std::getenv("CRT_EXACT_SLAB") != nullptr) ? 1u : 0u;
    W.pair_walk = (CRT_PAIR_WALK && !W.exact_slab && std::getenv("CRT_NO_PAIR_WALK") == nullptr) ? 1u : 0u;
}
static bool u16_entries(const crt_scene* s) { return (s->num_dnodes << kNodeFShift) <= 65536; }

static size_t partial_budget() {
    if (const char* e = std::getenv("CRT_PARTIAL_MB"))
        return static_cast<size_t>(std::max(1, std::atoi(e))) << 20;
    return size_t{4} << 30;
}

#ifndef CRT_CHUNK_MIN
#define CRT_CHUNK_MIN 4
#endif
uint32_t sample_chunk_len(uint32_t spp) {
    return std::max<uint32_t>(CRT_CHUNK_MIN, (spp + 191) / 192);
}

static int pass_pool(int device, hipMemPool_t* out) {
    static std::mutex mu;
    static hipMemPool_t pools[kMaxDevices] = {};
    std::lock_guard<std::mutex> lk(mu);
    if (device < 0 || device >= kMaxDevices) return fail(CRT_E_NODEVICE, "pass scratch pool: device out of range");
    if (!pools[device]) {
        hipMemPoolProps props{};
        props.allocType = hipMemAllocationTypePinned;
        props.handleTypes = hipMemHandleTypeNone;
        props.location.type = hipMemLocationTypeDevice;
        props.location.id = device;
        hipMemPool_t pool = nullptr;
        uint64_t keep = UINT64_MAX;
        hipError_t e = hipMemPoolCreate(&pool, &props);
        if (e == hipSuccess) {
            e = hipMemPoolSetAttribute(pool, hipMemPoolAttrReleaseThreshold, &keep);
            if (e != hipSuccess) (void)hipMemPoolDestroy(pool);
        }
        if (e != hipSuccess) {
            (void)hipGetLastError();
            return fail(CRT_E_HIP, std::string("pass scratch pool on device ") + std::to_string(device) + ": " +
                                       hipGetErrorString(e));
        }
        pools[device] = pool;
    }
    *out = pools[device];
    return CRT_OK;
}

template <typename SE, bool GSTACK, bool LSCENE, int PM, bool W5 = false>
static int launch_render(const crt_scene* s, int device, const crt_camera* cam, const dev::Work& w0,
                         size_t lds, double* d_rgb, hipStream_t stream, crt_render_stats* count_stats,
                         const RenderPass* pass) {
    const DeviceCopy& c = s->dev[device];
    dev::Work W = w0;
    lds = render_lds_tail(W, lds, GSTACK, LSCENE, PM, W5);
    constexpr int kThreads = dev::kBlock;
    const bool masked = pass && pass->blocks;
    const void* kfn = masked ? reinterpret_cast<const void*>(dev::render_kernel<SE, GSTACK, LSCENE, false, PM, W5, true>)
                             : reinterpret_cast<const void*>(dev::render_kernel<SE, GSTACK, LSCENE, false, PM, W5>);
    const uint64_t pixels = static_cast<uint64_t>(W.owned_rows) * cam->image_w;
    const uint32_t spp = cam->samples_per_pixel;
    W.chunk_len = sample_chunk_len(spp);
    W.chunks = (spp + W.chunk_len - 1) / W.chunk_len;
    uint32_t full_chunks = 0;
    double inv_done = 0;
    hipMemPool_t pool = nullptr;
    if (pass) {
        const int rc = pass_pool(device, &pool);
        if (rc) return rc;
    }
    auto scratch = [&](void** p, size_t bytes) {
        return pool ? hipMallocFromPoolAsync(p, bytes, pool, stream) : hipMallocAsync(p, bytes, stream);
    };
    if (pass) {
        const uint32_t end = pass->first + pass->count;
        W.s0 = pass->first;
        W.chunks = (end + W.chunk_len - 1) / W.chunk_len - pass->first / W.chunk_len;
        full_chunks = end / W.chunk_len - pass->first / W.chunk_len;
        inv_done = 1 / static_cast<double>(end);
    }
    constexpr uint64_t kMaxTiles = 65535;
    const uint64_t tiles_x_all = (static_cast<uint64_t>(cam->image_w) + dev::kTileW - 1) / dev::kTileW;
    const uint64_t tiles_y_all = (static_cast<uint64_t>(W.owned_rows) + dev::kTileH - 1) / dev::kTileH;
    const uint64_t tile_bytes = 64ull * 3 * sizeof(double) * W.chunks;
    const uint64_t cap = std::max<uint64_t>(1, partial_budget() / tile_bytes);
    const uint32_t bx = static_cast<uint32_t>(std::min({tiles_x_all, kMaxTiles, cap}));
    const uint32_t by = static_cast<uint32_t>(std::min({tiles_y_all, kMaxTiles, std::max<uint64_t>(1, cap / bx)}));
    int cus = 0, per_cu = 0;
    HIP_TRY(hipDeviceGetAttribute(&cus, hipDeviceAttributeMultiprocessorCount, device));
    HIP_TRY(hipOccupancyMaxActiveBlocksPerMultiprocessor(&per_cu, kfn, kThreads, lds));
    constexpr uint32_t kWavesPerBlock = kThreads / 64;
    uint64_t resident = static_cast<uint64_t>(std::max(1, cus)) * std::max(1, per_cu);
    if (const char* e = std::getenv("CRT_GRID_BLOCKS"))
        resident = std::max<uint64_t>(1, std::min<uint64_t>(resident, static_cast<uint64_t>(std::max(1, std::atoi(e)))));
    auto knob = [](const char* name, uint32_t dflt) {
        const char* e = std::getenv(name);
        return e ? static_cast<uint32_t>(std::max(0, std::min(4096, std::atoi(e)))) : dflt;
    };

    double* partial = nullptr;
    SE* gstack = nullptr;
    dev::Counters* ctr = nullptr;
    const bool count = count_stats != nullptr;
    const uint64_t band_px = std::min<uint64_t>(static_cast<uint64_t>(bx) * dev::kTileW, cam->image_w) *
                             std::min<uint64_t>(static_cast<uint64_t>(by) * dev::kTileH, W.owned_rows);
    if (!count)
        HIP_TRY(scratch(reinterpret_cast<void**>(&partial), band_px * 3 * W.chunks * sizeof(double)));
    if (GSTACK) {
        size_t bytes = gstack_levels(s) * resident * dev::kBlock * sizeof(SE);
        HIP_TRY(scratch(reinterpret_cast<void**>(&gstack), bytes));
    }
    if (count) {
        HIP_TRY(hipMallocAsync(reinterpret_cast<void**>(&ctr), sizeof(dev::Counters), stream));
        HIP_TRY(hipMemsetAsync(ctr, 0, sizeof(dev::Counters), stream));
    }
    uint32_t* queue = nullptr;
    HIP_TRY(scratch(reinterpret_cast<void**>(&queue), 256));
    W.queue = queue;
    uint32_t* active = nullptr;
    if (masked)
        HIP_TRY(scratch(reinterpret_cast<void**>(&active), (static_cast<size_t>(bx) * by + 1) * sizeof(uint32_t)));
    dev::SceneView S = view_of(c);
    dev::CamView C = cam_view(cam);
    hipEvent_t e0 = nullptr, e1 = nullptr;
    if (count) {
        HIP_TRY(hipEventCreate(&e0));
        HIP_TRY(hipEventCreate(&e1));
        HIP_TRY(hipEventRecord(e0, stream));
    }
    for (uint64_t ty0 = 0; ty0 < tiles_y_all; ty0 += by) {
        for (uint64_t tx0 = 0; tx0 < tiles_x_all; tx0 += bx) {
            W.col0 = static_cast<uint32_t>(tx0 * dev::kTileW);
            W.k0 = static_cast<uint32_t>(ty0 * dev::kTileH);
            W.bw = static_cast<uint32_t>(std::min<uint64_t>(static_cast<uint64_t>(bx) * dev::kTileW, cam->image_w - W.col0));
            W.bh = static_cast<uint32_t>(std::min<uint64_t>(static_cast<uint64_t>(by) * dev::kTileH, W.owned_rows - W.k0));
            W.tiles_x = (W.bw + dev::kTileW - 1) / dev::kTileW;
            W.tiles_y = (W.bh + dev::kTileH - 1) / dev::kTileH;
            W.tiles = W.tiles_x * W.tiles_y;
            const uint64_t q_tiles = masked && pass->hint ? std::min<uint64_t>(pass->hint, W.tiles) : W.tiles;
            const uint64_t blocks = std::max<uint64_t>(
                1, std::min<uint64_t>(resident, (q_tiles * W.chunks + kWavesPerBlock - 1) / kWavesPerBlock));
            const uint64_t per_lane = q_tiles * W.chunks / (blocks * kWavesPerBlock);
            const uint32_t k_auto = per_lane >= 60 ? static_cast<uint32_t>(std::min<uint64_t>(7, per_lane / 15)) : 3u;
            W.item_chunks = std::max<uint32_t>(1, knob("CRT_ITEM_CHUNKS", k_auto));
            const uint32_t tail_auto = static_cast<uint32_t>(std::max<uint64_t>(
                W.chunks / 9, std::min<uint64_t>(W.chunks, static_cast<uint64_t>(W.chunks) * 30 / std::max<uint64_t>(1, per_lane))));
            const uint32_t tail_want = std::min(W.chunks, knob("CRT_TAIL_CHUNKS", W.item_chunks > 1 ? tail_auto : 0));
            W.groups = (W.chunks - tail_want) / W.item_chunks;
            W.bulk_chunks = W.groups * W.item_chunks;
            W.tail_chunks = W.chunks - W.bulk_chunks;
            const uint64_t bulk_items = static_cast<uint64_t>(W.tiles) * W.groups;
            const uint64_t items = bulk_items + static_cast<uint64_t>(W.tiles) * W.tail_chunks;
            if (items >= 0xffffffffull) return fail(CRT_E_INVALID, "band too large for one launch");
            W.n_items = static_cast<uint32_t>(items);
            W.bulk_items = static_cast<uint32_t>(bulk_items);
            W.segments = knob("CRT_XCD_QUEUES", LSCENE ? 0 : 1) ? 8u : 1u;
            if (!masked) HIP_TRY(hipMemsetAsync(queue, 0, 8 * sizeof(uint32_t), stream));
#if CRT_WATCHDOG
            {
                void* wd = nullptr;
                HIP_TRY(hipGetSymbolAddress(&wd, HIP_SYMBOL(dev::crt_wd_deadline)));
                HIP_TRY(hipMemsetAsync(wd, 0, sizeof(unsigned long long), stream));
            }
#endif
            if (count) {
                hipLaunchKernelGGL((dev::render_kernel<SE, GSTACK, LSCENE, true, PM, W5>), dim3(static_cast<uint32_t>(blocks)),
                                   dim3(dev::kBlock), lds, stream, S, C, W, partial, gstack, ctr, nullptr);
                HIP_TRY(hipGetLastError());
            } else if (masked) {
                const uint32_t ftx = static_cast<uint32_t>(tiles_x_all);
                hipLaunchKernelGGL(dev::active_list_kernel, dim3(1), dim3(dev::kListThreads), 0, stream, pass->blocks, W, ftx,
                                   pass->first, active);
                HIP_TRY(hipGetLastError());
                hipLaunchKernelGGL((dev::render_kernel<SE, GSTACK, LSCENE, false, PM, W5, true>), dim3(static_cast<uint32_t>(blocks)),
                                   dim3(dev::kBlock), lds, stream, S, C, W, partial, gstack, ctr, active);
                HIP_TRY(hipGetLastError());
                hipLaunchKernelGGL(dev::accumulate_masked_kernel, dim3((W.tiles + 3) / 4), dim3(256), 0, stream, partial,
                                   pass->sum, pass->noise, d_rgb, pass->blocks, W, cam->image_w, ftx, full_chunks,
                                   pass->first + pass->count, inv_done);
                HIP_TRY(hipGetLastError());
            } else {
                hipLaunchKernelGGL((dev::render_kernel<SE, GSTACK, LSCENE, false, PM, W5>), dim3(static_cast<uint32_t>(blocks)),
                                   dim3(dev::kBlock), lds, stream, S, C, W, partial, gstack, ctr, nullptr);
                HIP_TRY(hipGetLastError());
                const uint64_t rb = (static_cast<uint64_t>(W.bw) * W.bh + 255) / 256;
                if (pass)
                    hipLaunchKernelGGL(dev::accumulate_kernel, dim3(static_cast<uint32_t>(rb)), dim3(256), 0, stream, partial,
                                       pass->sum, pass->noise, d_rgb, W, cam->image_w, full_chunks, inv_done);
                else
                    hipLaunchKernelGGL(dev::resolve_kernel, dim3(static_cast<uint32_t>(rb)), dim3(256), 0, stream, partial,
                                       d_rgb, W, cam->image_w, cam->image_h, C.inv_spp);
                HIP_TRY(hipGetLastError());
            }
        }
    }
    if (count) HIP_TRY(hipEventRecord(e1, stream));
    if (partial) HIP_TRY(hipFreeAsync(partial, stream));
    HIP_TRY(hipFreeAsync(queue, stream));
    if (active) HIP_TRY(hipFreeAsync(active, stream));
    if (gstack) HIP_TRY(hipFreeAsync(gstack, stream));
    if (count) {
        dev::Counters h{};
        HIP_TRY(hipMemcpyAsync(&h, ctr, sizeof h, hipMemcpyDeviceToHost, stream));
        HIP_TRY(hipStreamSynchronize(stream));
        HIP_TRY(hipFreeAsync(ctr, stream));
        HIP_TRY(hipStreamSynchronize(stream));
        float ms = 0;
        HIP_TRY(hipEventElapsedTime(&ms, e0, e1));
        (void)hipEventDestroy(e0);
        (void)hipEventDestroy(e1);
        count_stats->samples = pixels * cam->samples_per_pixel;
        count_stats->rays = h.rays;
        count_stats->nodes_visited = h.nodes;
        count_stats->sphere_tests = h.sphere_tests;
        count_stats->parallelogram_tests = h.quad_tests;
        count_stats->kernel_ms = ms;
        count_stats->ticks_walk = h.cyc_walk;
        count_stats->ticks_leaf = h.cyc_leaf;
        count_stats->ticks_shade = h.cyc_shade;
        count_stats->ticks_total = h.cyc_total;
        count_stats->wave_iters_walk = h.it_walk;
        count_stats->wave_iters_leaf = h.it_leaf;
        count_stats->wave_iters_shade = h.it_shade;
        count_stats->ticks_tail = h.cyc_tail;
        count_stats->slow_node_tests = h.slow_nodes;
        count_stats->wave_iters_slow = h.it_slow;
        count_stats->candidate_tests = h.cand;
        count_stats->wave_iters_candidates = h.it_cand;
        if (std::getenv("CRT_DEBUG_COUNTERS"))
            std::fprintf(stderr, "crt counters: rays %llu nodes %llu sphere_tests %llu quad_tests %llu it_walk %llu "
                         "it_leaf %llu it_shade %llu rounds %llu walkers/round %.2f leaves/round %.2f done/round %.2f "
"shade_rounds %llu; wave time: walk %.3f leaf %.3f shade %.3f draw %.3f init %.3f\n", h.rays, h.nodes, h.sphere_tests, h.quad_tests, h.it_walk,
                         h.it_leaf, h.it_shade, h.rounds, double(h.round_walkers) / double(h.rounds ? h.rounds : 1),
                         double(h.round_leaves) / double(h.rounds ? h.rounds : 1),
                         double(h.round_done) / double(h.rounds ? h.rounds : 1), h.shade_rounds,
                         double(h.cyc_walk) / double(h.cyc_total), double(h.cyc_leaf) / double(h.cyc_total),
                         double(h.cyc_shade) / double(h.cyc_total), double(h.cyc_draw) / double(h.cyc_total),
                         double(h.cyc_init) / double(h.cyc_total));
    }
    return CRT_OK;
}

template <typename SE>
static Layout render_layout(const crt_scene* s, dev::Work& W) {
    Layout L;
    const size_t stack_bytes = align16(static_cast<size_t>(s->depth + 1) * dev::kBlock * sizeof(SE));
    W.bytes_nodes = static_cast<uint32_t>(align16(s->num_dnodes * sizeof(DevNodeF)));
    W.bytes_refs = W.spheres_f32 ? 0u : static_cast<uint32_t>(align16(s->num_prims * 4));
    W.bytes_spheres = static_cast<uint32_t>(align16(s->num_spheres * (W.spheres_f32 ? sizeof(DevSpherePair)
                                                                                         : sizeof(DevSphere))));
    W.bytes_quads = static_cast<uint32_t>(align16(s->num_quads * sizeof(DevQuad)));
    W.bytes_quadf = W.quads_f32 ? static_cast<uint32_t>(s->num_quads * (W.quads_flat ? sizeof(DevQuadBox) : sizeof(DevQuadF)))
                                : 0u;
    const size_t scene_bytes = static_cast<size_t>(W.bytes_nodes) + W.bytes_refs + W.bytes_spheres + W.bytes_quads +
                               W.bytes_quadf;
    const uint32_t level = static_cast<uint32_t>(dev::kBlock * sizeof(SE));
    W.sentinel = static_cast<uint32_t>(s->num_dnodes - 1) << kNodeFShift;
    L.stack_bytes = stack_bytes;
    L.level = level;
    L.all_nodes = s->num_dnodes * sizeof(DevNodeF);
    const bool force_global = std::getenv("CRT_NO_LDS_SCENE") != nullptr;
    auto stack_at = [&](size_t data_bytes) { return static_cast<uint32_t>(std::max<size_t>(data_bytes, 2 * level) + 2 * level); };
    const size_t cam_bytes = align16(sizeof(dev::CamView));
    if (!force_global && stack_at(scene_bytes) + stack_bytes + cam_bytes <= kLdsSceneBudget) {
        W.lds_nodes = 0;
        W.lds_refs = W.lds_nodes + W.bytes_nodes;
        W.lds_spheres = W.lds_refs + W.bytes_refs;
        W.lds_quads = W.lds_spheres + W.bytes_spheres;
        W.lds_quadf = W.lds_quads + W.bytes_quads;
        W.lds_sph64 = W.lds_quadf + W.bytes_quadf;
        const size_t budget5 = kLdsBudget5;
        const bool w5 = (64 * dev::kManyWaves * 4) % dev::kBlock == 0 && (W.sphere_only || W.quads_flat) && std::getenv("CRT_FOUR_WAVES") == nullptr &&
                        stack_at(scene_bytes) + stack_bytes + cam_bytes + (W.sphere_only ? kAccBytes : 0) +
                            (W.quads_flat ? kInvBytes : 0) <= budget5;
        const size_t budget = w5 ? budget5 : kLdsSceneBudget;
        const uint32_t sph64 = static_cast<uint32_t>(s->num_spheres * sizeof(DevSphere));
        if (W.spheres_f32 && stack_at(scene_bytes + sph64) + stack_bytes + cam_bytes + (w5 ? kAccBytes : 0) <= budget)
            W.bytes_sph64 = sph64;
        W.lds_stack = stack_at(scene_bytes + W.bytes_sph64);
        L.cls = kQueryLdsScene;
        L.w5 = w5;
        L.lds = W.lds_stack + stack_bytes;
        L.budget = budget;
        return L;
    }
    const size_t per_block = kLdsPerBlock;
    L.budget = per_block;
    const bool no_top = std::getenv("CRT_NO_LDS_TOP") != nullptr;
    const size_t all_nodes = L.all_nodes;
    auto top_bytes = [&](size_t room) {
        return no_top ? 0u : static_cast<uint32_t>(std::min(all_nodes, room / (2 * sizeof(DevNodeF)) * (2 * sizeof(DevNodeF))));
    };
    if (stack_bytes <= kLdsStackBudget && stack_at(0) + stack_bytes + kInvBytes + cam_bytes <= per_block &&
        std::getenv("CRT_FORCE_GSTACK") == nullptr) {
        const size_t taken = stack_bytes + 2 * level + kInvBytes + cam_bytes;
        W.ntop = top_bytes(per_block - taken);
        W.lds_nodes = 0;
        W.lds_stack = stack_at(align16(W.ntop));
        L.cls = kQueryLdsStack;
        L.lds = W.lds_stack + stack_bytes;
        return L;
    }
    W.ntop = top_bytes(per_block - cam_bytes);
    W.lds_nodes = 0;
    L.cls = kQueryHbmStack;
    L.lds = W.ntop;
    return L;
}

template <typename SE>
static int dispatch_render(const crt_scene* s, int device, const crt_camera* cam, dev::Work W,
                           double* d_rgb, hipStream_t st, crt_render_stats* count_stats, const RenderPass* pass) {
    const Layout L = render_layout<SE>(s, W);
    const int pm = render_prim_mode(W, L.cls);
    switch (L.cls) {
    case kQueryLdsScene:
        if (pm == 0)
            return L.w5 ? launch_render<SE, false, true, 0, true>(s, device, cam, W, L.lds, d_rgb, st, count_stats, pass)
                        : launch_render<SE, false, true, 0, false>(s, device, cam, W, L.lds, d_rgb, st, count_stats, pass);
        if (pm == 2)
            return L.w5 ? launch_render<SE, false, true, 2, true>(s, device, cam, W, L.lds, d_rgb, st, count_stats, pass)
                        : launch_render<SE, false, true, 2, false>(s, device, cam, W, L.lds, d_rgb, st, count_stats, pass);
        return launch_render<SE, false, true, 1>(s, device, cam, W, L.lds, d_rgb, st, count_stats, pass);
    case kQueryLdsStack:
        if (pm == 0) return launch_render<SE, false, false, 0>(s, device, cam, W, L.lds, d_rgb, st, count_stats, pass);
        return launch_render<SE, false, false, 1>(s, device, cam, W, L.lds, d_rgb, st, count_stats, pass);
    default:
        if (pm == 0) return launch_render<SE, true, false, 0>(s, device, cam, W, L.lds, d_rgb, st, count_stats, pass);
        return launch_render<SE, true, false, 1>(s, device, cam, W, L.lds, d_rgb, st, count_stats, pass);
    }
}

static int tiling_work(const crt_camera* cam, const crt_tiling* t, dev::Work& W) {
    crt_tiling tl{1, 1, 0, 0};
    if (t) tl = *t;
    if (tl.flags & ~CRT_TILING_PACKED) return fail(CRT_E_INVALID, "unknown tiling flags");
    if (tl.row_block == 0 || tl.tile_count == 0 || tl.tile_index >= tl.tile_count)
        return fail(CRT_E_INVALID, "bad tiling");
    W = dev::Work{};
    W.row_block = tl.row_block;
    W.tile_count = tl.tile_count;
    W.tile_index = tl.tile_index;
    W.owned_rows = count_owned(cam->image_h, tl.row_block, tl.tile_count, tl.tile_index);
    W.packed = (tl.flags & CRT_TILING_PACKED) ? 1u : 0u;
    W.rb_shift = 32;
    for (uint32_t sh = 0; sh < 31; ++sh)
        if ((1u << sh) == W.row_block) W.rb_shift = sh;
    return CRT_OK;
}

int device_render(const crt_scene* s, int device, const crt_camera* cam, const crt_tiling* t,
                  double* d_rgb, void* stream, crt_render_stats* count_stats, const RenderPass* pass) {
    int rc = check_device(device);
    if (rc) return rc;
    if (!s->dev[device].valid)
        return fail(CRT_E_NOT_UPLOADED, "scene not uploaded to device " + std::to_string(device));
    if (cam->image_w == 0 || cam->image_h == 0) return fail(CRT_E_INVALID, "empty image");
    if (static_cast<uint64_t>(cam->image_w) * cam->image_h >= 0xffffffffull)
        return fail(CRT_E_INVALID, "image has more than 2^32-1 pixels");
    dev::Work W;
    rc = tiling_work(cam, t, W);
    if (rc) return rc;
    DeviceGuard g(device);
    if (W.owned_rows == 0 || cam->samples_per_pixel == 0) {
        if (count_stats) *count_stats = crt_render_stats{};
        if (cam->samples_per_pixel == 0 && d_rgb && W.owned_rows) {
            std::vector<double> nanrow(static_cast<size_t>(cam->image_w) * 3,
                                       std::numeric_limits<double>::quiet_NaN());
            for (uint32_t k = 0; k < W.owned_rows; ++k) {
                const size_t row = owned_to_frame_row(k, W.row_block, W.tile_count, W.tile_index, W.packed != 0);
                HIP_TRY(hipMemcpyAsync(d_rgb + row * cam->image_w * 3, nanrow.data(),
                                       nanrow.size() * 8, hipMemcpyHostToDevice,
                                       static_cast<hipStream_t>(stream)));
            }
            HIP_TRY(hipStreamSynchronize(static_cast<hipStream_t>(stream)));
        }
        return CRT_OK;
    }
    class_flags(s, flags_of(s->dev[device]), s->dev[device].f32_ok, true, W);
    W.tmin32 = static_cast<float>(cam->t_min);
    W.count_spec = std::getenv("CRT_COUNT_SPEC") != nullptr ? 1u : 0u;
    W.round_counters = std::getenv("CRT_ROUND_COUNTERS") != nullptr ? 1u : 0u;
    hipStream_t st = static_cast<hipStream_t>(stream);
    if (count_stats) HIP_TRY(hipStreamCreate(&st));
    int r;
    if (u16_entries(s))
        r = dispatch_render<uint16_t>(s, device, cam, W, d_rgb, st, count_stats, pass);
    else
        r = dispatch_render<uint32_t>(s, device, cam, W, d_rgb, st, count_stats, pass);
    if (count_stats) (void)hipStreamDestroy(st);
    return r;
}

static int ref_prim_table(const crt_scene* cs, int device, const uint32_t** out);

int device_closest_hits(crt_scene* s, int device, const double* rays, size_t n, double t_min,
                        double t_max, crt_hit* out) {
// ... 751 lines not shown
```

### cpp_raytracer_amd/csrc/crt_host.cpp

```cpp
#include <algorithm>
#include <atomic>
#include <sys/mman.h>
#include <chrono>
#include <cmath>
#include <cstdint>
#include <cstdio>
#include <cstdlib>
#include <cstring>
#include <limits>
#include <memory>
#include <numbers>
#include <numeric>
#include <optional>
#include <random>
#include <string>
#include <thread>
#include <vector>

#include "crt_internal.h"
#include "crt_prims.h"

namespace crt {

void* big_alloc(size_t bytes) {
    constexpr size_t kHuge = size_t{2} << 20, kMin = size_t{32} << 20;
    static const bool off = std::getenv("CRT_NO_HUGEPAGES") != nullptr;
    if (bytes < kMin || off) {
        void* p = std::malloc(std::max<size_t>(bytes, 1));
        if (!p) throw std::bad_alloc();
        return p;
    }
    const size_t rounded = (bytes + kHuge - 1) / kHuge * kHuge;
    void* p = std::aligned_alloc(kHuge, rounded);
    if (!p) throw std::bad_alloc();
    (void)madvise(p, rounded, MADV_HUGEPAGE);
    return p;
}
void big_free(void* p, size_t) noexcept { std::free(p); }

static thread_local std::string g_last_error;

int fail(int code, const std::string& msg) {
    g_last_error = msg;
    return code;
}
void clear_error() { g_last_error.clear(); }

struct V3 {
    double x = 0, y = 0, z = 0;
    double operator[](int a) const { return a == 0 ? x : (a == 1 ? y : z); }
};
static inline V3 add(V3 a, V3 b) { return {a.x + b.x, a.y + b.y, a.z + b.z}; }
static inline V3 sub(V3 a, V3 b) { return {a.x - b.x, a.y - b.y, a.z - b.z}; }
static inline V3 neg(V3 a) { return {-a.x, -a.y, -a.z}; }
static inline V3 mul(V3 a, double d) { return {a.x * d, a.y * d, a.z * d}; }
static inline V3 divv(V3 a, double d) { return mul(a, 1 / d); }
static inline double dot(V3 a, V3 b) { return a.x * b.x + a.y * b.y + a.z * b.z; }
static inline V3 cross(V3 a, V3 b) {
    return {a.y * b.z - a.z * b.y, a.z * b.x - a.x * b.z, a.x * b.y - a.y * b.x};
}
static inline double mag2(V3 a) { return a.x * a.x + a.y * a.y + a.z * a.z; }
static inline double mag(V3 a) { return std::sqrt(a.x * a.x + a.y * a.y + a.z * a.z); }
static inline V3 unit(V3 a) { return divv(a, mag(a)); }
static inline V3 v3(const double* p) { return {p[0], p[1], p[2]}; }
static inline void put(double* p, V3 a) { p[0] = a.x; p[1] = a.y; p[2] = a.z; }

using prim::gfmax;
using prim::gfmin;

struct Iv {
    double min, max;
    double size() const { return max - min; }
    void merge(const Iv& o) { min = gfmin(min, o.min); max = gfmax(max, o.max); }
    void merge(double d) { min = gfmin(min, d); max = gfmax(max, d); }
    double mid() const { return std::midpoint(min, max); }
};
constexpr double kInf = std::numeric_limits<double>::infinity();
struct Box3 {
    Iv a[3] = {{kInf, -kInf}, {kInf, -kInf}, {kInf, -kInf}};
    void merge(const Box3& o) { for (int i = 0; i < 3; ++i) a[i].merge(o.a[i]); }
    void merge(V3 p) { a[0].merge(p.x); a[1].merge(p.y); a[2].merge(p.z); }
    V3 centroid() const { return {a[0].mid(), a[1].mid(), a[2].mid()}; }
    double area() const {
        return 2 * (a[0].size() * a[0].size() + a[1].size() * a[1].size() +
                    a[2].size() * a[2].size());
    }
};
static Box3 box_of(const double* b) {
    Box3 r;
    for (int i = 0; i < 3; ++i) r.a[i] = {b[2 * i], b[2 * i + 1]};
    return r;
}
static void box_put(double* b, const Box3& r) {
    for (int i = 0; i < 3; ++i) { b[2 * i] = r.a[i].min; b[2 * i + 1] = r.a[i].max; }
}


static void emit_object(const crt_object& o, Prim* out) {
    const uint32_t np = prim::object_prims(o);
    for (uint32_t j = 0; j < np; ++j) {
        out[j].kind = prim::object_prim(o, j, out[j].v, out[j].box);
        out[j].material = o.material;
    }
}

// ... 1535 lines not shown
    if (rc) return rc;
    rc = check_pass(fn, s, cam, first_sample, num_samples, d_sum);
    if (rc) return rc;
    if (static_cast<uint64_t>(cam->image_w) * cam->image_h > 0x7fffffffull)
        return fail(CRT_E_INVALID, std::string(fn) + ": frame has more than 2^31-1 pixels");
    if (d_blocks && first_sample + num_samples >= CRT_BLOCK_STOPPED)
        return fail(CRT_E_INVALID, std::string(fn) + ": sample counts must stay below 2^31");
    (void)active_hint;
    return device_render_lens_pass(s, device, cam, lens, first_sample, num_samples, d_sum, d_noise, d_rgb, d_blocks, stream);
}

int crt_lens_centre_rays_async(int device, const crt_camera* cam, const crt_lens* lens, double* d_rays, void* stream) {
    clear_error();
    const std::string who = "crt_lens_centre_rays_async: ";
    const int rc = check_lens(who, false, nullptr, cam, lens, false);
    if (rc) return rc;
    if (!d_rays) return fail(CRT_E_INVALID, who + "d_rays is null (the output is required)");
    if (static_cast<uint64_t>(cam->image_w) * cam->image_h > 0x7fffffffull)
        return fail(CRT_E_INVALID, who + "frame has more than 2^31-1 pixels");
    return device_lens_centre_rays(device, cam, lens, d_rays, stream);
}

int crt_lens_features_async(const crt_scene* s, int device, const crt_camera* cam, const crt_lens* lens,
                            crt_feature* d_feat, void* stream) {
    clear_error();
    const std::string who = "crt_lens_features_async: ";
    const int rc = check_lens(who, true, s, cam, lens, false);
    if (rc) return rc;
    if (!d_feat) return fail(CRT_E_INVALID, who + "d_feat is null (the output is required)");
    if (static_cast<uint64_t>(cam->image_w) * cam->image_h > 0x7fffffffull)
        return fail(CRT_E_INVALID, who + "frame has more than 2^31-1 pixels");
    return device_lens_features(s, device, cam, lens, d_feat, stream);
}

int crt_render_lens_passes(crt_scene* s, int device, const crt_camera* cam, const crt_lens* lens,
                           const crt_adaptive_params* adaptive, const crt_denoise_params* denoise, crt_denoised_fn fn,
                           void* user, double* h_noisy, double* h_rgb, uint32_t* h_block_samples,
                           uint64_t* samples_rendered) {
    clear_error();
    if (samples_rendered) *samples_rendered = 0;
    const std::string who = "crt_render_lens_passes: ";
    int rc = check_lens(who, true, s, cam, lens, true);
    if (rc) return rc;
    if (!h_rgb) return fail(CRT_E_INVALID, who + "h_rgb is null (the output is required)");
    if (denoise) {
        rc = check_denoise_params("crt_render_lens_passes", denoise);
        if (rc) return rc;
    } else if (h_noisy) {
        return fail(CRT_E_INVALID, who + "h_noisy must be null without denoise (h_rgb is the unfiltered frame)");
    }
    if (adaptive) {
        if (adaptive->flags & ~CRT_PROGRESS_PREVIEW)
            return fail(CRT_E_INVALID, who + "unknown adaptive flags (CRT_PROGRESS_PREVIEW or 0)");
        if (adaptive->reserved != 0) return fail(CRT_E_INVALID, who + "adaptive reserved must be 0");
        if (!(adaptive->threshold >= 0) || !std::isfinite(adaptive->threshold))
            return fail(CRT_E_INVALID, who + "threshold must be finite and >= 0");
    }
    if (static_cast<uint64_t>(cam->image_w) * cam->image_h > 0x7fffffffull)
        return fail(CRT_E_INVALID, who + "frame has more than 2^31-1 pixels");
    return render_lens_passes(s, device, cam, lens, adaptive, denoise, fn, user, h_noisy, h_rgb, h_block_samples,
                              samples_rendered);
}

int crt_closest_hits(crt_scene* s, int device, const double* rays, size_t n, double t_min,
                     double t_max, crt_hit* out) {
    clear_error();
    if (!s || (n && (!rays || !out))) return fail(CRT_E_INVALID, "crt_closest_hits: null argument");
    return device_closest_hits(s, device, rays, n, t_min, t_max, out);
}

int crt_render_guard(crt_scene* s, int device, uint64_t* schlick_undecided, int reset) {
    clear_error();
    if (!s || !schlick_undecided) return fail(CRT_E_INVALID, "crt_render_guard: null argument");
    return device_guard(s, device, schlick_undecided, reset != 0);
}

int crt_launch_plan(const crt_scene* s, uint32_t kernel, crt_launch_plan_info* out) {
    clear_error();
    if (!s || !out) return fail(CRT_E_INVALID, "crt_launch_plan: null argument");
    if (kernel > CRT_PLAN_RADIANCE) return fail(CRT_E_INVALID, "crt_launch_plan: unknown kernel");
    return device_launch_plan(const_cast<crt_scene*>(s), kernel, out);
}

}
```

### cpp_raytracer_amd/csrc/crt_internal.h

```cpp
#pragma once

#include <cstddef>
#include <algorithm>
#include <cstdint>
#include <memory>
#include <mutex>
#include <type_traits>
#include <utility>
#include <string>
#include <thread>
#include <vector>

#include "../../include/crt_render.h"
#include "crt_quad_filter.h"

namespace crt {

constexpr int kMaxDevices = 16;

void* big_alloc(size_t bytes);
void big_free(void* p, size_t bytes) noexcept;
template <typename T>
struct NoInitAlloc : std::allocator<T> {
    using value_type = T;
// ... 117 lines not shown
    }
    if (!(std::fabs(sp.r) <= kF32SphereMax)) bad = true;
    cx = static_cast<float>(sp.c[0]);
    cy = static_cast<float>(sp.c[1]);
    cz = static_cast<float>(sp.c[2]);
    r2e = static_cast<float>(sp.r * sp.r * (1 + 0x1p-14) + dc2 * 0x1p22);
    return bad;
}

CRT_HD bool node_record(const DevNode& n, uint32_t i, DevNodeF& f) {
    bool bad = false;
    for (int k = 0; k < 6; ++k) {
        f.b[k] = static_cast<float>(n.b[k]);
        if (!std::isinf(n.b[k]) && !(std::fabs(n.b[k]) <= kF32BoundMax)) bad = true;
    }
    if (n.count == 0 && n.index == n.flags + 1 && !(n.flags & 1u)) {
        f.w0 = n.axis;
        f.w1 = n.flags << kNodeFShift;
    } else if (n.count == 0) {
        f.w0 = 0;
        f.w1 = kLeafFlagF;
    } else if (n.count == kSentinelCount) {
        f.w0 = (i << kNodeFShift) | 3u;
        f.w1 = kSentinelW1;
    } else {
        f.w0 = n.index;
        f.w1 = kLeafFlagF | n.count;
    }
    return bad;
}

CRT_HD bool regroup_leaf(const DevNode& nd, size_t k, DevQuadBox* quadbox) {
    if (nd.count == 0 || nd.count > 32 || nd.count == kSentinelCount) return false;
    if (k == 1 && !(nd.b[0] <= nd.b[1])) return false;
    DevQuadBox tmp[32];
    uint32_t n = 0, groups[3] = {0, 0, 0};
    bool bad = false;
    for (uint32_t axis = 0; axis < 3; ++axis)
        for (uint32_t j = 0; j < nd.count; ++j) {
            const DevQuadBox& r = quadbox[nd.index + j];
            uint32_t flat = 3;
            for (uint32_t q = 0; q < 3 && flat == 3; ++q)
                if (r.b[2 * q] == r.b[2 * q + 1]) flat = q;
            if (flat == 3) bad = true;
            if (flat == axis) {
                tmp[n] = r;
                tmp[n].pad[0] = j;
                ++n;
                ++groups[axis];
            }
        }
    if (n != nd.count) return bad;
    tmp[0].pad[1] = groups[0] | groups[1] << 8;
    for (uint32_t j = 0; j < n; ++j) quadbox[nd.index + j] = tmp[j];
    return bad;
}

struct DeviceCopy {
    bool valid = false;
    void* base = nullptr;
    size_t bytes = 0;
    DevNode* nodes = nullptr;
    DevNodeF* fnodes = nullptr;
    bool f32_ok = false;
    uint32_t* refs = nullptr;
    DevSphere* spheres = nullptr;
    DevSpherePair* spair = nullptr;
    bool spheres_f32_ok = false;
    uint32_t* sphere_mat = nullptr;
    DevQuad* quads = nullptr;
    DevQuadF* quadf = nullptr;
    bool quads_f32_ok = false;
    DevQuadBox* quadbox = nullptr;
    bool quads_flat_ok = false;
    uint32_t* quad_mat = nullptr;
    DevMaterial* mats = nullptr;
    DevMaterial* sphere_mrec = nullptr;
    DevMaterial* quad_mrec = nullptr;
    double* partial = nullptr;
    size_t partial_bytes = 0;
    unsigned long long* counters = nullptr;
    unsigned long long* guard = nullptr;
    uint32_t* ref_prim = nullptr;
};

struct Prim {
    uint32_t kind;
    uint32_t material;
    double v[15];
    double box[6];
};

}

struct crt_scene {
    crt::BigVec<crt_material> materials;
    crt::BigVec<crt_object> objects;
    crt::BigVec<crt::Prim> prims;
    crt::BigVec<double> pbox;
    crt::BigVec<crt_bvh_node> nodes;
    crt::BigVec<uint32_t> order;
    crt::BigVec<crt::DevNode> dnodes;
    crt::BigVec<uint32_t> refs;
    crt::BigVec<crt::DevSphere> spheres;
    crt::BigVec<uint32_t> sphere_mat;
    crt::BigVec<crt::DevQuad> quads;
    crt::BigVec<uint32_t> quad_mat;
    crt::BigVec<crt::DevMaterial> dmats;
    size_t num_objects = 0, num_materials = 0, num_prims = 0;
    size_t num_dnodes = 0, num_spheres = 0, num_quads = 0, num_dmats = 0;
    int image_device = -1;
    uint32_t depth = 0;
    uint32_t max_leaf = 0;
    double build_ms = 0;
    bool linear = false;
    bool exact_slab = false;
    crt::DeviceCopy dev[crt::kMaxDevices];
    std::mutex dev_mu[crt::kMaxDevices];
    crt::BigVec<char> image;
    bool staged = false;
    bool image_f32_ok = false, image_spheres_f32_ok = false, image_quads_f32_ok = false, image_quads_flat_ok = false;
    std::mutex mu;
};

namespace crt {
enum DevArray { kArrNodes, kArrFNodes, kArrRefs, kArrSpheres, kArrSpherePairs, kArrSphereMat, kArrQuads,
                kArrQuadF, kArrQuadBox, kArrQuadMat, kArrMats, kArrSphereMrec, kArrQuadMrec, kArrGuard,
                kArrCount };
static_assert(kArrFNodes + 1 < kArrGuard, "an array must follow the f32 nodes in the device allocation");
inline size_t device_layout(const crt_scene* s, size_t off[kArrCount + 1]) {
    const size_t n_nodes = s->num_dnodes, n_sp = s->num_spheres, n_q = s->num_quads;
    const size_t bytes[kArrCount] = {
        n_nodes * sizeof(DevNode), n_nodes * sizeof(DevNodeF), s->num_prims * 4, n_sp * sizeof(DevSphere),
        n_sp * sizeof(DevSpherePair), n_sp * 4, n_q * sizeof(DevQuad), n_q * sizeof(DevQuadF),
        n_q * sizeof(DevQuadBox), n_q * 4, std::max<size_t>(1, s->num_dmats) * sizeof(DevMaterial),
        n_sp * sizeof(DevMaterial), n_q * sizeof(DevMaterial), 64};
    size_t o = 0;
    for (int i = 0; i < kArrCount; ++i) {
        off[i] = o;
        o = (o + bytes[i] + 255) & ~size_t(255);
    }
    off[kArrCount] = o;
    return o;
}

int fail(int code, const std::string& msg);
void clear_error();

int device_upload(crt_scene* s, int device);
void device_release(crt_scene* s);
struct RenderPass {
    uint32_t first, count;
    double* sum;
    double* noise;
    uint32_t* blocks = nullptr;
    uint32_t hint = 0;
};
uint32_t sample_chunk_len(uint32_t spp);
int device_render(const crt_scene* s, int device, const crt_camera* cam, const crt_tiling* t,
                  double* d_rgb, void* stream, crt_render_stats* count_stats,
                  const RenderPass* pass = nullptr);
int device_noise_estimate(int device, const double* d_noise, size_t pixels, uint32_t spp,
                          uint32_t samples_done, double* sum_se, double* sum_mean, void* stream);
bool adaptive_tiling_ok(const crt_tiling* t);
int device_adaptive_update(int device, const crt_camera* cam, const crt_tiling* t, const double* d_noise,
                           uint32_t* d_blocks, uint32_t samples_done, double threshold, uint32_t min_samples,
                           uint32_t* active_blocks, void* stream);
int device_frame_from_sums(const crt_camera* cam, const crt_tiling* t, double* d_sum, uint32_t* d_blocks,
                           double* d_rgb, void* stream);
bool device_ppm8(const double* d_rgb, uint64_t px, uint8_t* d_out, uint32_t* d_redo, uint32_t redo_cap, void* stream);
bool device_redo_gather(const double* d_rgb, const uint32_t* d_list, uint32_t n, double* d_out, void* stream);
bool device_scale(const double* d_sum, double* d_out, uint64_t count, double factor, void* stream);
int device_closest_hits(crt_scene* s, int device, const double* rays, size_t n, double t_min,
                        double t_max, crt_hit* out);
int device_trace(const crt_scene* s, int device, const double* d_rays, size_t n, const double* d_tmax,
                 const crt_trace_params* prm, crt_hit* d_hits, uint32_t* d_occluded, void* stream);
int device_trace_host(crt_scene* s, int device, const double* rays, size_t n, const double* tmax,
                      const crt_trace_params* prm, crt_hit* hits, uint32_t* occluded);
int device_radiance(const crt_scene* s, int device, const double* d_rays, size_t n, const uint32_t* d_states,
                    const crt_radiance_params* prm, double* d_rgb, void* stream);
int device_radiance_host(crt_scene* s, int device, const double* rays, size_t n, const uint32_t* states,
                         const crt_radiance_params* prm, double* rgb);
int device_launch_plan(crt_scene* s, uint32_t kernel, crt_launch_plan_info* out);
int device_camera_rays(int device, const crt_camera* cam, const crt_tiling* t, uint32_t first_sample,
                       uint32_t num_samples, double* d_rays, uint32_t* d_states, void* stream);
int device_probe_rays(int device, const double* d_points, const double* d_normals, size_t n,
                      const crt_probe_params* prm, double* d_rays, uint32_t* d_states, void* stream);
int device_probes(const crt_scene* s, int device, const double* d_points, const double* d_normals, size_t n,
                  const crt_probe_params* prm, double* d_coeff, void* stream);
int device_probes_host(crt_scene* s, int device, const double* points, const double* normals, size_t n,
                       const crt_probe_params* prm, double* coeff);
int device_sh_eval(int device, const double* d_coeff, size_t num_probes, const uint32_t* d_index,
                   const double* d_dirs, size_t m, uint32_t what, double* d_rgb, void* stream);
int device_lens_rays(int device, const crt_camera* cam, const crt_lens* lens, uint32_t first_sample,
                     uint32_t num_samples, double* d_rays, uint32_t* d_states, void* stream);
int device_render_lens(const crt_scene* s, int device, const crt_camera* cam, const crt_lens* lens, double* d_rgb,
                       void* stream);
int device_render_lens_host(crt_scene* s, int device, const crt_camera* cam, const crt_lens* lens, double* rgb);
int device_render_lens_pass(const crt_scene* s, int device, const crt_camera* cam, const crt_lens* lens, uint32_t first,
                            uint32_t count, double* d_sum, double* d_noise, double* d_rgb, uint32_t* d_blocks,
                            void* stream);
int device_lens_centre_rays(int device, const crt_camera* cam, const crt_lens* lens, double* d_rays, void* stream);
int device_lens_features(const crt_scene* s, int device, const crt_camera* cam, const crt_lens* lens, crt_feature* d_feat,
                         void* stream);
int device_render_features(const crt_scene* s, int device, const crt_camera* cam, const crt_tiling* t,
                           crt_feature* d_feat, void* stream);
int device_pixel_variance(int device, const crt_camera* cam, const crt_tiling* t, const double* d_noise,
                          const uint32_t* d_blocks, uint32_t samples_done, double* d_var, void* stream);
int device_denoise(int device, uint32_t w, uint32_t h, const double* d_rgb, const double* d_var,
                   const crt_feature* d_feat, const crt_denoise_params* prm, double* d_out, double* d_var_out,
                   void* stream);
constexpr size_t kDenoiseStateBytes = 32, kDenoiseGuideBytes = 64;
int device_denoise_pack(int device, uint64_t pixels, const double* d_rgb, const double* d_var,
                        const crt_feature* d_feat, void* d_state, void* d_guide, void* stream);
int device_denoise_filter(int device, uint32_t w, uint32_t h, void* d_state, void* d_state_tmp, const void* d_guide,
                          const crt_denoise_params* prm, double* d_out, double* d_var_out, void* stream);
int device_check(int device);
int device_pass_pool(int device, void** pool);
int device_count(int* n);
const char* device_build_info();
int device_guard(crt_scene* s, int device, uint64_t* schlick_undecided, bool reset);
int device_build_bvh(crt_scene* s, uint32_t num_buckets, uint32_t max_leaf, int device,
                     const BigVec<double>& boxes);
void device_bind_copy(crt_scene* s, int device, void* base, size_t total);
int device_image(crt_scene* s, int device, void* host, size_t bytes);
struct DeviceTree {
    crt_bvh_node* nodes = nullptr;
    uint32_t* order = nullptr;
    uint32_t nnodes = 0, depth = 0, max_leaf = 0;
};
int device_build_tree(size_t n, const double* d_pb, uint32_t num_buckets, uint32_t max_leaf, DeviceTree& out);
void device_tree_free(DeviceTree& t);
int device_create_scene(crt_scene* s, const crt_material* materials, size_t num_materials,
                        const crt_object* objects, size_t num_objects, const crt_bvh_params& prm, int device,
                        bool* host_path);
int validate_scene(const crt_material* materials, size_t nm, const crt_object* objects, size_t no,
                   size_t* nprims, size_t* nspheres, bool* boxes);
int device_ppm_values(int device, const double* d_rgb, size_t n, int32_t* h_values, void* stream);
void ppm_pixel_host(const double rgb[3], int32_t out[3]);

int render_multi(crt_scene* s, const crt_camera* cam, int num_devices, double* h_rgb,
                 crt_render_stats* stats);
int render_multi_ppm(crt_scene* s, const crt_camera* cam, int num_devices, int32_t* h_values,
                     crt_render_stats* stats);
int render_progressive(crt_scene* s, const crt_camera* cam, int num_devices, uint32_t samples_per_pass,
                       uint32_t flags, crt_progress_fn fn, void* user, double* h_rgb,
                       uint32_t* samples_done);
int render_adaptive(crt_scene* s, const crt_camera* cam, int num_devices, const crt_adaptive_params* prm,
                    crt_adaptive_fn fn, void* user, double* h_rgb, uint32_t* h_block_samples,
                    uint64_t* samples_rendered);
int render_denoised(crt_scene* s, int device, const crt_camera* cam, const crt_adaptive_params* adaptive,
                    const crt_denoise_params* denoise, double* h_noisy, double* h_rgb, uint64_t* samples_rendered);
int render_denoised_devices(crt_scene* s, const crt_camera* cam, int num_devices, const crt_adaptive_params* adaptive,
                            const crt_denoise_params* denoise, crt_denoised_fn fn, void* user, double* h_noisy,
                            double* h_rgb, uint32_t* h_block_samples, uint64_t* samples_rendered);
int render_lens_passes(crt_scene* s, int device, const crt_camera* cam, const crt_lens* lens,
                       const crt_adaptive_params* adaptive, const crt_denoise_params* denoise, crt_denoised_fn fn,
                       void* user, double* h_noisy, double* h_rgb, uint32_t* h_block_samples, uint64_t* samples_rendered);
}
```

### include/crt_render.h

```cpp
#ifndef CRT_RENDER_H
#define CRT_RENDER_H

#include <stddef.h>
#include <stdint.h>

#ifdef __cplusplus
extern "C" {
#endif

#define CRT_ABI_VERSION 2

#define CRT_OK 0
#define CRT_E_INVALID (-1)
#define CRT_E_HIP (-2)
#define CRT_E_NODEVICE (-3)
#define CRT_E_NOT_UPLOADED (-4)
#define CRT_E_ALLOC (-5)

enum {
    CRT_LAMBERTIAN = 1,
    CRT_METAL = 2,
    CRT_DIELECTRIC = 3,
    CRT_DIFFUSE_LIGHT = 4
};
// ... 291 lines not shown

int crt_probes_async(const crt_scene* scene, int device, const double* d_points, const double* d_normals,
                     size_t n, const crt_probe_params* params, double* d_coeff, void* stream);

int crt_probes(crt_scene* scene, int device, const double* points, const double* normals, size_t n,
               const crt_probe_params* params, double* coeff);

#define CRT_SH_RADIANCE   0u
#define CRT_SH_IRRADIANCE 1u
#define CRT_SH_A0 3.141592653589793
#define CRT_SH_A1 2.0943951023931953
#define CRT_SH_A2 0.7853981633974483
int crt_sh_eval_async(int device, const double* d_coeff, size_t num_probes, const uint32_t* d_index,
                      const double* d_dirs, size_t m, uint32_t what, double* d_rgb, void* stream);

#define CRT_LENS_PINHOLE       0u
#define CRT_LENS_ORTHOGRAPHIC  1u
#define CRT_LENS_EQUIRECT      2u
#define CRT_LENS_FISHEYE       3u
#define CRT_LENS_CUBE          4u
typedef struct crt_lens {
    uint32_t kind, flags;
    double origin[3];
    double right[3], up[3], forward[3];
    double extent_x, extent_y;
    uint64_t batch_pixels;
} crt_lens;

int crt_lens_rays_async(int device, const crt_camera* cam, const crt_lens* lens, uint32_t first_sample,
                        uint32_t num_samples, double* d_rays, uint32_t* d_states, void* stream);

int crt_render_lens_async(const crt_scene* scene, int device, const crt_camera* cam, const crt_lens* lens,
                          double* d_rgb, void* stream);

int crt_render_lens(crt_scene* scene, int device, const crt_camera* cam, const crt_lens* lens, double* rgb);

int crt_render_lens_pass_async(const crt_scene* scene, int device, const crt_camera* cam, const crt_lens* lens,
                               uint32_t first_sample, uint32_t num_samples, double* d_sum, double* d_noise,
                               double* d_rgb, uint32_t* d_blocks, uint32_t active_hint, void* stream);

int crt_lens_centre_rays_async(int device, const crt_camera* cam, const crt_lens* lens, double* d_rays, void* stream);

int crt_lens_features_async(const crt_scene* scene, int device, const crt_camera* cam, const crt_lens* lens,
                            crt_feature* d_feat, void* stream);

int crt_render_lens_passes(crt_scene* scene, int device, const crt_camera* cam, const crt_lens* lens,
                           const crt_adaptive_params* adaptive, const crt_denoise_params* denoise,
                           crt_denoised_fn fn, void* user, double* h_noisy, double* h_rgb,
                           uint32_t* h_block_samples, uint64_t* samples_rendered);

int crt_ppm_values(int device, const double* d_rgb, size_t n, int32_t* h_values, void* stream);

int crt_ppm_write(const char* path, uint32_t w, uint32_t h, const int32_t* values);

int crt_render_guard(crt_scene* scene, int device, uint64_t* schlick_undecided, int reset);

enum { CRT_PLAN_RENDER = 0, CRT_PLAN_TRACE = 1, CRT_PLAN_RADIANCE = 2 };
enum { CRT_PLAN_LDS_SCENE = 0, CRT_PLAN_LDS_STACK = 1, CRT_PLAN_HBM_STACK = 2 };
#define CRT_PLAN_ABSENT 0xffffffffu
typedef struct crt_launch_plan_info {
    uint32_t kernel;
    uint32_t klass;
    uint32_t entry_bytes;
    uint32_t five_waves;
    uint32_t prim_mode;
    uint32_t plain_route;
    uint32_t depth;
    uint32_t block;
    uint64_t num_nodes;
    uint32_t stack_bytes, level, sentinel;
    uint32_t hbm_stack_levels;
    uint32_t lds_nodes, lds_refs, lds_spheres, lds_quads, lds_quadf, lds_sph64, lds_stack;
    uint32_t bytes_nodes, bytes_refs, bytes_spheres, bytes_quads, bytes_quadf, bytes_sph64;
    uint32_t ntop, all_nodes;
    uint32_t lds_cam, lds_acc, lds_inv64;
    uint32_t bytes_cam, bytes_acc, bytes_inv64;
    uint32_t total_lds;
    uint32_t budget;
    uint32_t spheres_f32, quads_f32, quads_flat, f32_ok;
    uint32_t reserved[9];
} crt_launch_plan_info;
int crt_launch_plan(const crt_scene* scene, uint32_t kernel, crt_launch_plan_info* out);

#ifdef __cplusplus
}
#endif

#endif
```

Baseline: 6714 Msamples/s.

## Replace per-lane BVH traversal stack with per-octant miss links in LDS

```diff
diff --git a/cpp_raytracer_amd/__init__.py b/cpp_raytracer_amd/__init__.py
--- a/cpp_raytracer_amd/__init__.py
+++ b/cpp_raytracer_amd/__init__.py
@@ -280,6 +280,26 @@
         p = _capi.LaunchPlan()
         check(lib().crt_launch_plan(self._h, int(k), C.byref(p)), "crt_launch_plan")
         return p
+
+    def walk_links(self) -> Optional[np.ndarray]:
+        n = C.c_size_t(0)
+        check(lib().crt_walk_links(self._h, None, 0, C.byref(n)), "crt_walk_links")
+        if n.value == 0:
+            return None
+        out = np.zeros((n.value, 8), np.uint16)
+        check(lib().crt_walk_links(self._h, out.ctypes.data, out.size, C.byref(n)), "crt_walk_links")
+        return out
+
+    def walk_links_valid(self, links: np.ndarray) -> bool:
+        t = np.ascontiguousarray(links, np.uint16)
+        ok = C.c_int(0)
+        check(lib().crt_walk_links_validate(self._h, t.ctypes.data, t.size, C.byref(ok)), "crt_walk_links_validate")
+        return bool(ok.value)
+
+    def last_walk(self, device: int = 0) -> str:
+        w = C.c_uint32(0)
+        check(lib().crt_last_walk(self._h, device, C.byref(w)), "crt_last_walk")
+        return ("none", "stack", "links")[w.value]
 
     def upload(self, device: int = 0) -> None:
         check(lib().crt_scene_upload(self._h, device), f"crt_scene_upload(device={device})")
diff --git a/cpp_raytracer_amd/_capi.py b/cpp_raytracer_amd/_capi.py
--- a/cpp_raytracer_amd/_capi.py
+++ b/cpp_raytracer_amd/_capi.py
@@ -248,6 +248,9 @@
     "crt_ppm_write": (C.c_int, [C.c_char_p, C.c_uint32, C.c_uint32, C.c_void_p]),
     "crt_render_guard": (C.c_int, [C.c_void_p, C.c_int, P(C.c_uint64), C.c_int]),
     "crt_launch_plan": (C.c_int, [C.c_void_p, C.c_uint32, P(LaunchPlan)]),
+    "crt_walk_links": (C.c_int, [C.c_void_p, C.c_void_p, C.c_size_t, P(C.c_size_t)]),
+    "crt_walk_links_validate": (C.c_int, [C.c_void_p, C.c_void_p, C.c_size_t, P(C.c_int)]),
+    "crt_last_walk": (C.c_int, [C.c_void_p, C.c_int, P(C.c_uint32)]),
 }
 
 
diff --git a/cpp_raytracer_amd/csrc/crt_device.hip b/cpp_raytracer_amd/csrc/crt_device.hip
--- a/cpp_raytracer_amd/csrc/crt_device.hip
+++ b/cpp_raytracer_amd/csrc/crt_device.hip
@@ -63,6 +63,9 @@
     uint32_t refs_lds, spheres_lds, quads_lds;
     uint32_t inv64_lds;
     unsigned long long* guard;
+    const uint16_t* links;
+    uint32_t links_lds;
+    uint32_t sentinel;
 };
 
 struct CamView {
@@ -96,6 +99,7 @@
     uint32_t lds_cam;
     uint32_t lds_acc;
     uint32_t lds_inv64;
+    uint32_t lds_links, bytes_links;
     uint32_t packed;
     uint32_t count_spec, round_counters;
     uint32_t f32_ok;
@@ -800,12 +804,20 @@
     return w;
 }
 
-template <typename SE, bool COUNT, bool EXACT, bool TOP, bool LS, bool GS, bool SPEC, bool INVL = false, bool G2 = true>
+typedef __attribute__((address_space(3))) const uint16_t LdsU16;
+__device__ __forceinline__ uint32_t link_at(uint32_t lbase, uint32_t cur) {
+    return *(LdsU16*)static_cast<uintptr_t>(lbase + (cur >> 1));
+}
+
+template <typename SE, bool COUNT, bool EXACT, bool TOP, bool LS, bool GS, bool SPEC, bool INVL = false, bool G2 = true,
+          bool LINK = false>
 __device__ __forceinline__ void walk(const SceneView& S, Stack<SE>& st, const double o[3], const double d[3],
                                      double tmin, float tmin32, Trav& R, LaneCounters& ctr) {
-    const ptrdiff_t stride = static_cast<ptrdiff_t>(st.stride);
-    SE* const empty = st.base - stride;
-    SE* tp = st.base + (static_cast<ptrdiff_t>(R.sp) - 1) * stride;
+    static_assert(!LINK || (LS && !GS && !TOP), "miss links are staged by the LDS-scene instances only");
+    const ptrdiff_t stride = LINK ? 0 : static_cast<ptrdiff_t>(st.stride);
+    SE* const empty = LINK ? nullptr : st.base - stride;
+    SE* tp = LINK ? nullptr : st.base + (static_cast<ptrdiff_t>(R.sp) - 1) * stride;
+    const uint32_t lbase = LINK ? S.links_lds + ((R.neg & 7u) << 1) : 0u;
     uint32_t cur = R.cur;
     uint32_t w0, w1;
     bool stop;
@@ -817,7 +829,7 @@
             NodeLines nd;
             node_lines(node64(S, cur), nd);
             const Uvec4 meta = nd.meta;
-            const uint32_t top = *tp;
+            const uint32_t top = LINK ? link_at(lbase, cur) : *tp;
             if (COUNT) {
                 if (meta.y != kSentinelCount) ctr.nodes++;
                 if (wave_leader()) ctr.it_walk++;
@@ -843,10 +855,10 @@
             const bool inner = enter & (meta.y == 0);
             const bool far_first = (R.neg >> meta.z) & 1u;
             const uint32_t left = meta.w << kNodeFShift, right = meta.x << kNodeFShift;
-            tp[stride] = static_cast<SE>(far_first ? left : right);
+            if (!LINK) tp[stride] = static_cast<SE>(far_first ? left : right);
             stop = enter ^ inner;
             cur = inner ? (far_first ? right : left) : top;
-            tp += inner ? stride : -stride;
+            if (!LINK) tp += inner ? stride : -stride;
             w0 = meta.x;
             w1 = meta.y == kSentinelCount ? kSentinelW1 : (kLeafFlagF | meta.y);
         } while (!stop);
@@ -860,7 +872,7 @@
                 fetch_nodef<TOP, LS>(S, cur, q0, q1);
                 w0 = q1.z;
                 w1 = q1.w;
-                const uint32_t top = *tp;
+                const uint32_t top = LINK ? link_at(lbase, cur) : *tp;
                 if (COUNT) {
                     if (w1 != kSentinelW1) ctr.nodes++;
                     if (wave_leader()) ctr.it_walk++;
@@ -887,20 +899,20 @@
                 }
                 const bool inner = enter & (w1 < kLeafFlagF);
                 const uint32_t near = w1 | (__builtin_amdgcn_ubfe(R.neg, w0, 1) << kNodeFShift);
-                tp[stride] = static_cast<SE>(near ^ (1u << kNodeFShift));
+                if (!LINK) tp[stride] = static_cast<SE>(near ^ (1u << kNodeFShift));
                 const bool reached = enter & !inner;
                 const bool park = reached & (!nopend | (!G2 && w1 == kSentinelW1));
                 pref = (reached & nopend) ? cur : pref;
                 pcur = park ? cur : pcur;
                 run = !park;
                 cur = inner ? near : top;
-                tp += inner ? stride : -stride;
+                if (!LINK) tp += inner ? stride : -stride;
             }
             nopend = pref == ~0u;
         } while (__ballot(nopend) != 0);
         if (!run) {
             cur = pcur;
-            tp += stride;
+            if (!LINK) tp += stride;
         }
         {
             const Uvec2 w = fetch_nodef_words<TOP, LS>(S, pref);
@@ -911,7 +923,7 @@
         R.first = w0;
         R.count = w1 & ~kLeafFlagF;
         R.cur = cur;
-        R.sp = static_cast<int32_t>(static_cast<uint32_t>(tp - empty)) / static_cast<int32_t>(st.stride);
+        if (!LINK) R.sp = static_cast<int32_t>(static_cast<uint32_t>(tp - empty)) / static_cast<int32_t>(st.stride);
         return;
     } else {
         do {
@@ -920,7 +932,7 @@
             fetch_nodef<TOP, LS>(S, cur, q0, q1);
             w0 = q1.z;
             w1 = q1.w;
-            const uint32_t top = *tp;
+            const uint32_t top = LINK ? link_at(lbase, cur) : *tp;
             if (COUNT) {
                 if (w1 != kSentinelW1) ctr.nodes++;
                 if (wave_leader()) ctr.it_walk++;
@@ -947,17 +959,17 @@
             }
             const bool inner = enter & (w1 < kLeafFlagF);
             const uint32_t near = w1 | (__builtin_amdgcn_ubfe(R.neg, w0, 1) << kNodeFShift);
-            tp[stride] = static_cast<SE>(near ^ (1u << kNodeFShift));
+            if (!LINK) tp[stride] = static_cast<SE>(near ^ (1u << kNodeFShift));
             stop = enter ^ inner;
             cur = inner ? near : top;
-            tp += inner ? stride : -stride;
+            if (!LINK) tp += inner ? stride : -stride;
         } while (!stop);
     }
     R.state = w1 == kSentinelW1 ? kDone : kLeaf;
     R.first = w0;
     R.count = w1 & ~kLeafFlagF;
     R.cur = cur;
-    R.sp = static_cast<int32_t>(static_cast<uint32_t>(tp - empty)) / static_cast<int32_t>(st.stride);
+    if (!LINK) R.sp = static_cast<int32_t>(static_cast<uint32_t>(tp - empty)) / static_cast<int32_t>(st.stride);
 }
 
 
@@ -1090,7 +1102,7 @@
     R.sp = static_cast<int32_t>(static_cast<uint32_t>(tp - empty)) / static_cast<int32_t>(st.stride);
 }
 
-template <typename SE, bool COUNT, bool TOP, bool LS, bool FAST = false, bool QONLY = false>
+template <typename SE, bool COUNT, bool TOP, bool LS, bool FAST = false, bool QONLY = false, bool LINK = false>
 __device__ __forceinline__ void leaf_step(const SceneView& S, Stack<SE>& st, const double o[3],
                                               const double d[3], double tmin, float tmin32, bool sphere_only, bool pairs,
                                               bool qfilter, bool qflat, Trav& R, LaneCounters& ctr) {
@@ -1248,7 +1260,7 @@
             }
         }
     }
-    R.state = R.sp < 0 ? kDone : kWalk;
+    R.state = (LINK ? R.cur == S.sentinel : R.sp < 0) ? kDone : kWalk;
 }
 
 __device__ __forceinline__ uint32_t owned_row(const Work& w, uint32_t k) {
@@ -1403,7 +1415,7 @@
     if constexpr ((kPrioWalk | kPrioLeaf | kPrioShade | kPrioInit) != 0) __builtin_amdgcn_s_setprio(P);
 }
 
-template <typename SE, bool GSTACK, bool LSCENE, bool COUNT, int PM, bool W5, bool MASK = false>
+template <typename SE, bool GSTACK, bool LSCENE, bool COUNT, int PM, bool W5, bool MASK = false, bool LINK = false>
 __global__ __launch_bounds__(kBlock) __attribute__((amdgpu_waves_per_eu(W5 ? kManyWaves : LSCENE ? CRT_WAVES_PER_EU_LDS : CRT_WAVES_PER_EU, 8))) void render_kernel(
     SceneView Sg, CamView C, Work W, double* __restrict__ partial, SE* __restrict__ gstack,
     Counters* __restrict__ counters, const uint32_t* __restrict__ active) {
@@ -1433,6 +1445,11 @@
             S.refs = reinterpret_cast<const uint32_t*>(smem + W.lds_refs);
             S.spheres = reinterpret_cast<const DevSphere*>(smem + W.lds_spheres);
         }
+        if (LINK) {
+            stage_lds(smem + W.lds_links, Sg.links, W.bytes_links);
+            S.links_lds = W.lds_links;
+            S.sentinel = W.sentinel;
+        }
         __syncthreads();
     } else if (W.ntop) {
         if (static_cast<uint32_t>(reinterpret_cast<uintptr_t>((LdsByte*)smem)) != 0) __builtin_trap();
@@ -1450,16 +1467,19 @@
     const uint32_t lane = threadIdx.x & 63;
     LaneCounters ctr{};
     const unsigned long long t_start = COUNT ? wall_clock64() : 0;
-    Stack<SE> st;
-    if (GSTACK) {
+    Stack<SE> st{};
+    if (LINK) {
+    } else if (GSTACK) {
         st.stride = gridDim.x * kBlock;
         st.base = gstack + (static_cast<size_t>(blockIdx.x) * kBlock + threadIdx.x) + 3 * static_cast<size_t>(st.stride);
     } else {
         st.base = reinterpret_cast<SE*>(smem + W.lds_stack) + threadIdx.x;
         st.stride = kBlock;
     }
-    st.base[-static_cast<ptrdiff_t>(st.stride)] = static_cast<SE>(W.sentinel);
-    st.base[-2 * static_cast<ptrdiff_t>(st.stride)] = static_cast<SE>(W.sentinel);
+    if (!LINK) {
+        st.base[-static_cast<ptrdiff_t>(st.stride)] = static_cast<SE>(W.sentinel);
+        st.base[-2 * static_cast<ptrdiff_t>(st.stride)] = static_cast<SE>(W.sentinel);
+    }
     uint32_t item_pos = 0, item_units = 0;
     const uint32_t q_tiles = MASK ? active[0] : W.tiles;
     uint32_t seg = blockIdx.x % W.segments, seg_tried = 0;
@@ -1567,8 +1587,8 @@
         if (start || cont) {
             trav_init(P.o, P.d, W.f32_ok != 0, R);
             const bool tok = kPair && pw && !(R.neg & kZeroDir);
-            st.base[-static_cast<ptrdiff_t>(st.stride)] = static_cast<SE>(W.sentinel | (tok ? kTokAlone : 0u));
-            if (!kFlatOnly) st.base[-2 * static_cast<ptrdiff_t>(st.stride)] = static_cast<SE>(W.sentinel | (tok ? kTokAlone : 0u));
+            if (!LINK) st.base[-static_cast<ptrdiff_t>(st.stride)] = static_cast<SE>(W.sentinel | (tok ? kTokAlone : 0u));
+            if (!LINK && !kFlatOnly) st.base[-2 * static_cast<ptrdiff_t>(st.stride)] = static_cast<SE>(W.sentinel | (tok ? kTokAlone : 0u));
             if (tok) R.cur = kTokAlone;
             if (kInvLds) {
                 uint32_t t = threadIdx.x;
@@ -1604,12 +1624,12 @@
             } else if (!W.exact_slab && __ballot(R.state == kWalk && (R.neg & kZeroDir)) == 0) {
                 if (R.state == kWalk) {
                     if (!COUNT || W.count_spec)
-                        walk<SE, COUNT, false, kTopTreelet && !LSCENE, LSCENE, GSTACK, true, kInvLds, !kFlatOnly>(S, st, P.o, P.d, C.t_min, tmin32, R, ctr);
+                        walk<SE, COUNT, false, kTopTreelet && !LSCENE, LSCENE, GSTACK, true, kInvLds, !kFlatOnly, LINK>(S, st, P.o, P.d, C.t_min, tmin32, R, ctr);
                     else
-                        walk<SE, COUNT, false, kTopTreelet && !LSCENE, LSCENE, GSTACK, false, kInvLds>(S, st, P.o, P.d, C.t_min, tmin32, R, ctr);
+                        walk<SE, COUNT, false, kTopTreelet && !LSCENE, LSCENE, GSTACK, false, kInvLds, true, LINK>(S, st, P.o, P.d, C.t_min, tmin32, R, ctr);
                 }
             } else {
-                if (R.state == kWalk) walk<SE, COUNT, true, kTopTreelet && !LSCENE, LSCENE, GSTACK, false>(S, st, P.o, P.d, C.t_min, tmin32, R, ctr);
+                if (R.state == kWalk) walk<SE, COUNT, true, kTopTreelet && !LSCENE, LSCENE, GSTACK, false, false, true, LINK>(S, st, P.o, P.d, C.t_min, tmin32, R, ctr);
             }
             if (COUNT) cw += static_cast<uint32_t>(wall_clock64());
             set_prio<kPrioLeaf>();
@@ -1618,7 +1638,7 @@
                 if (wave_leader()) atomicAdd(&counters->round_leaves, nl);
             }
             if (COUNT) cl -= static_cast<uint32_t>(wall_clock64());
-            if (R.state == kLeaf) leaf_step<SE, COUNT, kTopTreelet && !LSCENE, LSCENE, kFast, kFlatOnly>(S, st, P.o, P.d, C.t_min, tmin32, kSphOnly || (!kFlatOnly && W.sphere_only != 0), !kFlatOnly && W.spheres_f32 != 0, kFlatOnly || (!kSphOnly && W.quads_f32 != 0), kFlatOnly || (!kSphOnly && W.quads_flat != 0), R, ctr);
+            if (R.state == kLeaf) leaf_step<SE, COUNT, kTopTreelet && !LSCENE, LSCENE, kFast, kFlatOnly, LINK>(S, st, P.o, P.d, C.t_min, tmin32, kSphOnly || (!kFlatOnly && W.sphere_only != 0), !kFlatOnly && W.spheres_f32 != 0, kFlatOnly || (!kSphOnly && W.quads_f32 != 0), kFlatOnly || (!kSphOnly && W.quads_flat != 0), R, ctr);
             if (COUNT) cl += static_cast<uint32_t>(wall_clock64());
             const uint64_t pending = __ballot(R.state == kWalk);
             const uint64_t finished = __ballot(R.state == kDone);
@@ -2577,6 +2597,7 @@
     dev::SceneView v{c.nodes, c.fnodes, 0, c.refs, c.spheres, c.spair, 0, c.sphere_mat, c.quads, c.quad_mat,
                      c.mats, c.quadf, c.sphere_mrec, c.quad_mrec, 0, c.quadbox};
     v.guard = c.guard;
+    v.links = c.links;
     return v;
 }
 
@@ -2706,6 +2727,9 @@
     return CopyFlags{c.f32_ok, c.spheres_f32_ok, c.quads_f32_ok, c.quads_flat_ok};
 }
 
+static bool u16_entries(const crt_scene* s);
+static void bind_links(crt_scene* s, DeviceCopy& c);
+
 void device_bind_copy(crt_scene* s, int device, void* base, size_t total) {
     size_t off[kArrCount + 1];
     (void)device_layout(s, off);
@@ -2733,6 +2757,68 @@
     c.quad_mrec = reinterpret_cast<DevMaterial*>(b + off[kArrQuadMrec]);
     c.guard = reinterpret_cast<unsigned long long*>(b + off[kArrGuard]);
     c.valid = true;
+    bind_links(s, c);
+}
+
+static bool copy_nodes_host(const crt_scene* s, const DeviceCopy& c, std::vector<DevNode>& out) {
+    out.resize(s->num_dnodes);
+    return hipMemcpy(out.data(), c.nodes, out.size() * sizeof(DevNode), hipMemcpyDeviceToHost) == hipSuccess;
+}
+
+static const std::vector<uint16_t>& scene_links(crt_scene* s, const DeviceCopy* from) {
+    std::lock_guard<std::mutex> lk(s->mu);
+    if (s->links_built) return s->links;
+    if (u16_entries(s) && s->num_dnodes >= 2) {
+        if (s->image_device < 0) {
+            std::vector<DevNode> nodes(s->dnodes.begin(), s->dnodes.end());
+            (void)scene_walk_links(nodes.data(), nodes.size(), s->links);
+        } else if (from) {
+            std::vector<DevNode> nodes;
+            if (copy_nodes_host(s, *from, nodes)) (void)scene_walk_links(nodes.data(), nodes.size(), s->links);
+            else (void)hipGetLastError();
+        } else {
+            return s->links;
+        }
+    }
+    s->links_built = true;
+    return s->links;
+}
+
+const std::vector<uint16_t>& device_walk_links(crt_scene* s) { return scene_links(s, nullptr); }
+
+static void bind_links(crt_scene* s, DeviceCopy& c) {
+    c.links = nullptr;
+    c.links_bytes = 0;
+    std::vector<uint16_t> table = scene_links(s, &c);
+    if (table.empty()) return;
+    const size_t bytes = (table.size() * sizeof(uint16_t) + 15) & ~size_t(15);
+    table.resize(bytes / sizeof(uint16_t), 0);
+    void* d = nullptr;
+    if (hipMalloc(&d, bytes) != hipSuccess || hipMemcpy(d, table.data(), bytes, hipMemcpyHostToDevice) != hipSuccess) {
+        (void)hipGetLastError();
+        if (d) (void)hipFree(d);
+        return;
+    }
+    c.links = static_cast<uint16_t*>(d);
+    c.links_bytes = static_cast<uint32_t>(bytes);
+}
+
+int device_nodes_host(crt_scene* s, std::vector<DevNode>& out) {
+    out.clear();
+    if (!u16_entries(s)) return CRT_OK;
+    if (s->image_device < 0) {
+        out.assign(s->dnodes.begin(), s->dnodes.end());
+        return CRT_OK;
+    }
+    std::lock_guard<std::mutex> lk(s->dev_mu[s->image_device]);
+    const DeviceCopy& c = s->dev[s->image_device];
+    if (!c.valid) return fail(CRT_E_NOT_UPLOADED, "the scene's device copy is gone");
+    DeviceGuard g(s->image_device);
+    if (!copy_nodes_host(s, c, out)) {
+        (void)hipGetLastError();
+        return fail(CRT_E_HIP, "reading the scene's nodes back failed");
+    }
+    return CRT_OK;
 }
 
 int device_upload(crt_scene* s, int device) {
@@ -2798,6 +2884,7 @@
         DeviceGuard g(d);
         (void)hipFree(c.base);
         if (c.ref_prim) (void)hipFree(c.ref_prim);
+        if (c.links) (void)hipFree(c.links);
         c = DeviceCopy{};
     }
 }
@@ -2934,7 +3021,7 @@
     return CRT_OK;
 }
 
-template <typename SE, bool GSTACK, bool LSCENE, int PM, bool W5 = false>
+template <typename SE, bool GSTACK, bool LSCENE, int PM, bool W5 = false, bool LINK = false>
 static int launch_render(const crt_scene* s, int device, const crt_camera* cam, const dev::Work& w0,
                          size_t lds, double* d_rgb, hipStream_t stream, crt_render_stats* count_stats,
                          const RenderPass* pass) {
@@ -2943,8 +3030,8 @@
     lds = render_lds_tail(W, lds, GSTACK, LSCENE, PM, W5);
     constexpr int kThreads = dev::kBlock;
     const bool masked = pass && pass->blocks;
-    const void* kfn = masked ? reinterpret_cast<const void*>(dev::render_kernel<SE, GSTACK, LSCENE, false, PM, W5, true>)
-                             : reinterpret_cast<const void*>(dev::render_kernel<SE, GSTACK, LSCENE, false, PM, W5>);
+    const void* kfn = masked ? reinterpret_cast<const void*>(dev::render_kernel<SE, GSTACK, LSCENE, false, PM, W5, true, LINK>)
+                             : reinterpret_cast<const void*>(dev::render_kernel<SE, GSTACK, LSCENE, false, PM, W5, false, LINK>);
     const uint64_t pixels = static_cast<uint64_t>(W.owned_rows) * cam->image_w;
     const uint32_t spp = cam->samples_per_pixel;
     W.chunk_len = sample_chunk_len(spp);
@@ -3051,7 +3138,7 @@
             }
 #endif
             if (count) {
-                hipLaunchKernelGGL((dev::render_kernel<SE, GSTACK, LSCENE, true, PM, W5>), dim3(static_cast<uint32_t>(blocks)),
+                hipLaunchKernelGGL((dev::render_kernel<SE, GSTACK, LSCENE, true, PM, W5, false, LINK>), dim3(static_cast<uint32_t>(blocks)),
                                    dim3(dev::kBlock), lds, stream, S, C, W, partial, gstack, ctr, nullptr);
                 HIP_TRY(hipGetLastError());
             } else if (masked) {
@@ -3059,7 +3146,7 @@
                 hipLaunchKernelGGL(dev::active_list_kernel, dim3(1), dim3(dev::kListThreads), 0, stream, pass->blocks, W, ftx,
                                    pass->first, active);
                 HIP_TRY(hipGetLastError());
-                hipLaunchKernelGGL((dev::render_kernel<SE, GSTACK, LSCENE, false, PM, W5, true>), dim3(static_cast<uint32_t>(blocks)),
+                hipLaunchKernelGGL((dev::render_kernel<SE, GSTACK, LSCENE, false, PM, W5, true, LINK>), dim3(static_cast<uint32_t>(blocks)),
                                    dim3(dev::kBlock), lds, stream, S, C, W, partial, gstack, ctr, active);
                 HIP_TRY(hipGetLastError());
                 hipLaunchKernelGGL(dev::accumulate_masked_kernel, dim3((W.tiles + 3) / 4), dim3(256), 0, stream, partial,
@@ -3067,7 +3154,7 @@
                                    pass->first + pass->count, inv_done);
                 HIP_TRY(hipGetLastError());
             } else {
-                hipLaunchKernelGGL((dev::render_kernel<SE, GSTACK, LSCENE, false, PM, W5>), dim3(static_cast<uint32_t>(blocks)),
+                hipLaunchKernelGGL((dev::render_kernel<SE, GSTACK, LSCENE, false, PM, W5, false, LINK>), dim3(static_cast<uint32_t>(blocks)),
                                    dim3(dev::kBlock), lds, stream, S, C, W, partial, gstack, ctr, nullptr);
                 HIP_TRY(hipGetLastError());
                 const uint64_t rb = (static_cast<uint64_t>(W.bw) * W.bh + 255) / 256;
@@ -3081,6 +3168,7 @@
             }
         }
     }
+    c.last_walk = LINK ? CRT_WALK_LINKS : CRT_WALK_STACK;
     if (count) HIP_TRY(hipEventRecord(e1, stream));
     if (partial) HIP_TRY(hipFreeAsync(partial, stream));
     HIP_TRY(hipFreeAsync(queue, stream));
@@ -3200,6 +3288,18 @@
                            double* d_rgb, hipStream_t st, crt_render_stats* count_stats, const RenderPass* pass) {
     const Layout L = render_layout<SE>(s, W);
     const int pm = render_prim_mode(W, L.cls);
+    if constexpr (std::is_same_v<SE, uint16_t>) {
+        const DeviceCopy& c = s->dev[device];
+        const size_t table = s->num_dnodes * 16;
+        if (L.cls == kQueryLdsScene && L.w5 && (pm == 0 || pm == 2) && c.links &&
+            c.links_bytes >= align16(table) && table <= 2 * L.level + L.stack_bytes &&
+            std::getenv("CRT_NO_LINK_WALK") == nullptr) {
+            W.lds_links = static_cast<uint32_t>(W.lds_stack - 2 * L.level);
+            W.bytes_links = static_cast<uint32_t>(align16(table));
+            return pm == 0 ? launch_render<SE, false, true, 0, true, true>(s, device, cam, W, L.lds, d_rgb, st, count_stats, pass)
+                           : launch_render<SE, false, true, 2, true, true>(s, device, cam, W, L.lds, d_rgb, st, count_stats, pass);
+        }
+    }
     switch (L.cls) {
     case kQueryLdsScene:
         if (pm == 0)
diff --git a/cpp_raytracer_amd/csrc/crt_host.cpp b/cpp_raytracer_amd/csrc/crt_host.cpp
--- a/cpp_raytracer_amd/csrc/crt_host.cpp
+++ b/cpp_raytracer_amd/csrc/crt_host.cpp
@@ -19,8 +19,15 @@
 
 #include "crt_internal.h"
 #include "crt_prims.h"
+#include "crt_walk_links.h"
 
 namespace crt {
+
+bool scene_walk_links(const DevNode* nodes, size_t n, std::vector<uint16_t>& links) {
+    if (build_walk_links(nodes, n, links) && validate_walk_links(nodes, n, links.data())) return true;
+    links.clear();
+    return false;
+}
 
 void* big_alloc(size_t bytes) {
     constexpr size_t kHuge = size_t{2} << 20, kMin = size_t{32} << 20;
@@ -1722,4 +1729,40 @@
     return device_launch_plan(const_cast<crt_scene*>(s), kernel, out);
 }
 
-}
+int crt_walk_links(crt_scene* s, uint16_t* links, size_t capacity, size_t* num_nodes) {
+    clear_error();
+    if (!s || !num_nodes) return fail(CRT_E_INVALID, "crt_walk_links: null argument");
+    *num_nodes = 0;
+    const std::vector<uint16_t>& table = device_walk_links(s);
+    if (table.empty()) return CRT_OK;
+    *num_nodes = table.size() / kWalkLinkOctants;
+    if (!links) return CRT_OK;
+    if (capacity < table.size())
+        return fail(CRT_E_INVALID, "crt_walk_links: capacity must be at least " + std::to_string(table.size()));
+    std::memcpy(links, table.data(), table.size() * sizeof(uint16_t));
+    return CRT_OK;
+}
+
+int crt_walk_links_validate(crt_scene* s, const uint16_t* links, size_t entries, int* ok) {
+    clear_error();
+    if (!s || !links || !ok) return fail(CRT_E_INVALID, "crt_walk_links_validate: null argument");
+    *ok = 0;
+    std::vector<DevNode> nodes;
+    const int rc = device_nodes_host(s, nodes);
+    if (rc) return rc;
+    if (entries != nodes.size() * kWalkLinkOctants)
+        return fail(CRT_E_INVALID, "crt_walk_links_validate: entries must be " +
+                                       std::to_string(nodes.size() * kWalkLinkOctants));
+    *ok = validate_walk_links(nodes.data(), nodes.size(), links) ? 1 : 0;
+    return CRT_OK;
+}
+
+int crt_last_walk(const crt_scene* s, int device, uint32_t* walk) {
+    clear_error();
+    if (!s || !walk) return fail(CRT_E_INVALID, "crt_last_walk: null argument");
+    if (device < 0 || device >= kMaxDevices) return fail(CRT_E_NODEVICE, "crt_last_walk: device out of range");
+    *walk = s->dev[device].last_walk;
+    return CRT_OK;
+}
+
+}
diff --git a/cpp_raytracer_amd/csrc/crt_internal.h b/cpp_raytracer_amd/csrc/crt_internal.h
--- a/cpp_raytracer_amd/csrc/crt_internal.h
+++ b/cpp_raytracer_amd/csrc/crt_internal.h
@@ -223,6 +223,9 @@
     unsigned long long* counters = nullptr;
     unsigned long long* guard = nullptr;
     uint32_t* ref_prim = nullptr;
+    uint16_t* links = nullptr;
+    uint32_t links_bytes = 0;
+    mutable uint32_t last_walk = 0;
 };
 
 struct Prim {
@@ -261,6 +264,8 @@
     crt::BigVec<char> image;
     bool staged = false;
     bool image_f32_ok = false, image_spheres_f32_ok = false, image_quads_f32_ok = false, image_quads_flat_ok = false;
+    std::vector<uint16_t> links;
+    bool links_built = false;
     std::mutex mu;
 };
 
@@ -365,6 +370,9 @@
                      const BigVec<double>& boxes);
 void device_bind_copy(crt_scene* s, int device, void* base, size_t total);
 int device_image(crt_scene* s, int device, void* host, size_t bytes);
+int device_nodes_host(crt_scene* s, std::vector<DevNode>& out);
+const std::vector<uint16_t>& device_walk_links(crt_scene* s);
+bool scene_walk_links(const DevNode* nodes, size_t n, std::vector<uint16_t>& links);
 struct DeviceTree {
     crt_bvh_node* nodes = nullptr;
     uint32_t* order = nullptr;
diff --git a/cpp_raytracer_amd/csrc/crt_walk_links.h b/cpp_raytracer_amd/csrc/crt_walk_links.h
--- /dev/null
+++ b/cpp_raytracer_amd/csrc/crt_walk_links.h
@@ -0,0 +1,95 @@
+#pragma once
+
+#include <cstddef>
+#include <cstdint>
+#include <vector>
+
+#include "crt_internal.h"
+
+namespace crt {
+
+constexpr size_t kWalkLinkOctants = 8;
+inline bool walk_links_fit(size_t num_nodes) { return num_nodes >= 2 && (num_nodes << kNodeFShift) <= 65536; }
+
+inline bool walk_node_interior(const DevNode& n) { return n.count == 0 && n.index == n.flags + 1 && !(n.flags & 1u); }
+
+inline bool build_walk_links(const DevNode* nodes, size_t n, std::vector<uint16_t>& links) {
+    links.clear();
+    if (!walk_links_fit(n) || nodes[n - 1].count != kSentinelCount) return false;
+    const uint16_t sentinel = static_cast<uint16_t>((n - 1) << kNodeFShift);
+    links.assign(n * kWalkLinkOctants, sentinel);
+    std::vector<unsigned char> placed(n, 0);
+    placed[0] = 1;
+    for (size_t i = 0; i + 1 < n; ++i) {
+        const DevNode& nd = nodes[i];
+        if (!walk_node_interior(nd)) continue;
+        if (!placed[i]) {
+            if (i == 1) continue;
+            return false;
+        }
+        const size_t left = nd.flags, right = nd.index;
+        if (left <= i || right >= n - 1 || nd.axis > 2 || placed[left] || placed[right]) return false;
+        placed[left] = placed[right] = 1;
+        for (size_t o = 0; o < kWalkLinkOctants; ++o) {
+            const bool far_first = (o >> nd.axis) & 1u;
+            const size_t near = far_first ? right : left, far = far_first ? left : right;
+            links[near * kWalkLinkOctants + o] = static_cast<uint16_t>(far << kNodeFShift);
+            links[far * kWalkLinkOctants + o] = links[i * kWalkLinkOctants + o];
+        }
+    }
+    return true;
+}
+
+inline bool validate_walk_links(const DevNode* nodes, size_t n, const uint16_t* links) {
+    if (!walk_links_fit(n) || nodes[n - 1].count != kSentinelCount) return false;
+    const size_t sentinel = n - 1;
+    std::vector<uint32_t> order, rank(n), size(n), stack;
+    for (size_t o = 0; o < kWalkLinkOctants; ++o) {
+        order.clear();
+        stack.assign(1, 0u);
+        std::vector<unsigned char> seen(n, 0);
+        while (!stack.empty()) {
+            const uint32_t i = stack.back();
+            stack.pop_back();
+            if (i >= sentinel || seen[i]) return false;
+            seen[i] = 1;
+            rank[i] = static_cast<uint32_t>(order.size());
+            order.push_back(i);
+            const DevNode& nd = nodes[i];
+            if (!walk_node_interior(nd)) continue;
+            if (nd.axis > 2) return false;
+            const bool far_first = (o >> nd.axis) & 1u;
+            stack.push_back(far_first ? nd.flags : nd.index);
+            stack.push_back(far_first ? nd.index : nd.flags);
+        }
+        for (size_t k = order.size(); k-- > 0;) {
+            const uint32_t i = order[k];
+            size[i] = 1;
+            if (walk_node_interior(nodes[i])) size[i] += size[nodes[i].flags] + size[nodes[i].index];
+        }
+        for (size_t i = 0; i < n; ++i) {
+            const size_t link = links[i * kWalkLinkOctants + o];
+            if (link & ((size_t{1} << kNodeFShift) - 1)) return false;
+            const size_t t = link >> kNodeFShift;
+            if (t >= n) return false;
+            if (i == sentinel || !seen[i]) {
+                if (t != sentinel) return false;
+                continue;
+            }
+            const size_t after = static_cast<size_t>(rank[i]) + size[i];
+            const size_t want = after < order.size() ? order[after] : sentinel;
+            if (t != want) return false;
+            if (t != sentinel && rank[t] <= rank[i]) return false;
+        }
+        for (size_t i = 0; i < n; ++i) {
+            size_t cur = i, steps = 0;
+            while (cur != sentinel) {
+                if (++steps > n) return false;
+                cur = links[cur * kWalkLinkOctants + o] >> kNodeFShift;
+            }
+        }
+    }
+    return true;
+}
+
+}
diff --git a/include/crt_render.h b/include/crt_render.h
--- a/include/crt_render.h
+++ b/include/crt_render.h
@@ -397,6 +397,11 @@
 } crt_launch_plan_info;
 int crt_launch_plan(const crt_scene* scene, uint32_t kernel, crt_launch_plan_info* out);
 
+enum { CRT_WALK_NONE = 0, CRT_WALK_STACK = 1, CRT_WALK_LINKS = 2 };
+int crt_walk_links(crt_scene* scene, uint16_t* links, size_t capacity, size_t* num_nodes);
+int crt_walk_links_validate(crt_scene* scene, const uint16_t* links, size_t entries, int* ok);
+int crt_last_walk(const crt_scene* scene, int device, uint32_t* walk);
+
 #ifdef __cplusplus
 }
 #endif
```

New measurement: 6896 Msamples/s, median of 6. 2.7% higher.
